# hbaatz/nerf-tex

Hardware: AMD Instinct MI355X
Metric: ray-samples/sec (MLP+composite) at 800x800x64 (higher is better)
Workload: dtype f32; 1 GPU; carpet 800x800x64: 640000 all-hit rays x 64 samples per GPU (BASELINE configs[1]), ParamNerf n_parameters=[1, 6], seeded glorot weights, inputs resident in HBM, fused PE+MLP+composite; rays_per_gpu=640000, hit_rays_total=640000, samples_per_ray=64

## Files before the change

nerf_tex_amd/csrc/ntx_train.hip:

```cpp
#include "nerftex.h"

#include <hip/hip_runtime.h>

#include <algorithm>
#include <cmath>
#include <cstdint>
#include <cstdio>
#include <cstdlib>
#include <cstring>
#include <type_traits>
#include <vector>

#include "ntx_train_device.h"

extern "C" int ntx_set_error(int code, const char *fmt, ...);

#define TRAIN_TRY(expr)                                                                                  \
    do {                                                                                                 \
        hipError_t e_ = (expr);                                                                          \
        if (e_ != hipSuccess) return ntx_set_error(NTX_E_HIP, "%s: %s", #expr, hipGetErrorString(e_)); \
    } while (0)

namespace ntx_train {

constexpr int TM = 128;

struct GemmArgs {
    const float *A; int lda; const float *B; int ldb; float *C; int ldc;
    int M, N, K;
    const float *bias;
    const float *mask; int ldmask;
    int relu, accumulate;
    int k_chunk; long long split_stride;
    float *colsum;
    int aligned;
};

template <int n, bool FAST>
__device__ __forceinline__ void fetch_run(const float *g, bool row_ok, int first, int bound, float *r, bool aligned_ok = false) {
    if (FAST) {
        const f32x4 *v = reinterpret_cast<const f32x4 *>(g);
#pragma unroll
        for (int q = 0; q < n / 4; ++q) { const f32x4 x = v[q]; r[4 * q] = x.x; r[4 * q + 1] = x.y; r[4 * q + 2] = x.z; r[4 * q + 3] = x.w; }
    } else if (row_ok && first + n <= bound && aligned_ok) {
        const f32x4 *v = reinterpret_cast<const f32x4 *>(g);
#pragma unroll
        for (int q = 0; q < n / 4; ++q) { const f32x4 x = v[q]; r[4 * q] = x.x; r[4 * q + 1] = x.y; r[4 * q + 2] = x.z; r[4 * q + 3] = x.w; }
    } else {
#pragma unroll
        for (int q = 0; q < n; ++q) r[q] = (row_ok && first + q < bound) ? g[q] : 0.0f;
    }
}

template <bool A_KCONTIG, int TN_, int TK_>
__device__ __forceinline__ void gemm_body(const GemmArgs &g, int bx, int by, int bz) {
    constexpr int THREADS = TN_ * 2, WCOLS = TN_ / 64, LROWA = TM + 4, LROWB_ = TN_ + 4;
    constexpr int FA = TM * TK_ / THREADS;
    constexpr int FB = TN_ * TK_ / THREADS;
    constexpr int TPR = THREADS / TK_;
    static_assert(FA % 4 == 0 && FB % 4 == 0 && FA * (THREADS / TM) == TK_ && TPR * FB == TN_ && TPR * FA == TM, "panel split");
    __shared__ __attribute__((aligned(16))) float As[2][TK_][LROWA], Bs[2][TK_][LROWB_];
    const int lane = threadIdx.x & 63, wave = threadIdx.x >> 6;
    const int j0 = bx * TN_, i0 = by * TM;
    const int k_begin = bz * g.k_chunk;
    const int k_end = k_begin + g.k_chunk < g.K ? k_begin + g.k_chunk : g.K;
    float *C = g.C + (size_t)bz * (size_t)g.split_stride;
    f32x16 acc[2][2];
#pragma unroll
    for (int a = 0; a < 2; ++a)
#pragma unroll
        for (int b = 0; b < 2; ++b)
#pragma unroll
            for (int r = 0; r < 16; ++r) acc[a][b][r] = 0.0f;
    float ra[2][FA], rb[2][FB], cs[FB];
#pragma unroll
    for (int q = 0; q < FB; ++q) cs[q] = 0.0f;
    const bool want_colsum = !A_KCONTIG && g.colsum != nullptr && by == 0;
    const bool inner = g.aligned && i0 + TM <= g.M && j0 + TN_ <= g.N;
    const int a_row = A_KCONTIG ? (int)(threadIdx.x % TM) : (int)(threadIdx.x / TPR), a_off = A_KCONTIG ? (int)(threadIdx.x / TM) * FA : (int)(threadIdx.x % TPR) * FA;
    const int b_row = (int)(threadIdx.x / TPR), b_off = (int)(threadIdx.x % TPR) * FB;
    auto fetch = [&](int k0, float *fa, float *fb) {
        const bool al = g.aligned != 0;
        if (A_KCONTIG) fetch_run<FA, false>(g.A + (size_t)(i0 + a_row) * g.lda + k0 + a_off, i0 + a_row < g.M, k0 + a_off, k_end, fa, al);
        else fetch_run<FA, false>(g.A + (size_t)(k0 + a_row) * g.lda + i0 + a_off, k0 + a_row < k_end, i0 + a_off, g.M, fa, al);
        fetch_run<FB, false>(g.B + (size_t)(k0 + b_row) * g.ldb + j0 + b_off, k0 + b_row < k_end, j0 + b_off, g.N, fb, al);
    };
    auto stash = [&](int buf, const float *fa, const float *fb) {
        if (want_colsum) {
#pragma unroll
            for (int q = 0; q < FB; ++q) cs[q] += fb[q];
        }
        if (A_KCONTIG) {
#pragma unroll
            for (int q = 0; q < FA; ++q) As[buf][a_off + q][a_row] = fa[q];
        } else {
            f32x4 *d = reinterpret_cast<f32x4 *>(&As[buf][a_row][a_off]);
#pragma unroll
            for (int q = 0; q < FA / 4; ++q) d[q] = f32x4{fa[4 * q], fa[4 * q + 1], fa[4 * q + 2], fa[4 * q + 3]};
        }
        f32x4 *d = reinterpret_cast<f32x4 *>(&Bs[buf][b_row][b_off]);
#pragma unroll
        for (int q = 0; q < FB / 4; ++q) d[q] = f32x4{fb[4 * q], fb[4 * q + 1], fb[4 * q + 2], fb[4 * q + 3]};
    };
    const int n_panels = (k_end - k_begin + TK_ - 1) / TK_;
    const int n_full = inner ? (k_end - k_begin) / TK_ : 0;
    const int wi = (wave / WCOLS) * 64 + 2 * (lane & 31), wj = (wave % WCOLS) * 64 + 2 * (lane & 31), kh = lane >> 5;
    const bool wave_live = j0 + (wave % WCOLS) * 64 < g.N;
    auto compute = [&](int buf) {
        if (!wave_live) return;
        f32x2 av[2], bv[2];
        av[0] = *reinterpret_cast<const f32x2 *>(&As[buf][kh][wi]); bv[0] = *reinterpret_cast<const f32x2 *>(&Bs[buf][kh][wj]);
#pragma unroll
        for (int st = 0; st < TK_ / 2; ++st) {
            const int c = st & 1, n = c ^ 1;
            if (st + 1 < TK_ / 2) {
                const int kk = 2 * (st + 1) + kh;
                av[n] = *reinterpret_cast<const f32x2 *>(&As[buf][kk][wi]); bv[n] = *reinterpret_cast<const f32x2 *>(&Bs[buf][kk][wj]);
            }
            __builtin_amdgcn_sched_barrier(0);
            acc[0][0] = __builtin_amdgcn_mfma_f32_32x32x2f32(av[c].x, bv[c].x, acc[0][0], 0, 0, 0);
            acc[0][1] = __builtin_amdgcn_mfma_f32_32x32x2f32(av[c].x, bv[c].y, acc[0][1], 0, 0, 0);
            acc[1][0] = __builtin_amdgcn_mfma_f32_32x32x2f32(av[c].y, bv[c].x, acc[1][0], 0, 0, 0);
            acc[1][1] = __builtin_amdgcn_mfma_f32_32x32x2f32(av[c].y, bv[c].y, acc[1][1], 0, 0, 0);
            __builtin_amdgcn_sched_barrier(0);
        }
    };
    auto fetch_fast = [&](int k0, float *fa, float *fb) {
        const float *ga = A_KCONTIG ? g.A + (size_t)(i0 + a_row) * g.lda + k0 + a_off : g.A + (size_t)(k0 + a_row) * g.lda + i0 + a_off;
        fetch_run<FA, true>(ga, true, 0, 0, fa);
        fetch_run<FB, true>(g.B + (size_t)(k0 + b_row) * g.ldb + j0 + b_off, true, 0, 0, fb);
    };
    auto pipeline = [&](auto fast_tag, int first, int last) {
        constexpr bool FAST = decltype(fast_tag)::value;
        auto get = [&](int kt, float *fa, float *fb) { if (FAST) fetch_fast(k_begin + kt * TK_, fa, fb); else fetch(k_begin + kt * TK_, fa, fb); };
        if (first >= last) return;
        get(first, ra[0], rb[0]); stash(0, ra[0], rb[0]);
        if (first + 1 < last) get(first + 1, ra[1], rb[1]);
        __syncthreads();
        int kt = first;
        for (; kt + 3 < last; kt += 2) {
            get(kt + 2, ra[0], rb[0]); compute(0); stash(1, ra[1], rb[1]); __syncthreads();
            get(kt + 3, ra[1], rb[1]); compute(1); stash(0, ra[0], rb[0]); __syncthreads();
        }
        for (; kt < last; ++kt) {
            const int buf = (kt - first) & 1;
            if (kt + 2 < last) { if (buf) get(kt + 2, ra[1], rb[1]); else get(kt + 2, ra[0], rb[0]); }
            compute(buf);
            if (kt + 1 < last) { if (buf) stash(0, ra[0], rb[0]); else stash(1, ra[1], rb[1]); }
            __syncthreads();
        }
    };
    pipeline(std::true_type{}, 0, n_full);
    pipeline(std::false_type{}, n_full, n_panels);
    const bool whole = i0 + TM <= g.M && j0 + TN_ <= g.N && (g.ldc % 2 == 0) && (!g.mask || g.ldmask % 2 == 0) && ((uintptr_t)C % 8 == 0) && ((uintptr_t)g.mask % 8 == 0);
    const int j = j0 + (wave % WCOLS) * 64 + 2 * (lane & 31);
    const float bj0 = (g.bias && j < g.N) ? g.bias[j] : 0.0f, bj1 = (g.bias && j + 1 < g.N) ? g.bias[j + 1] : 0.0f;
#pragma unroll
    for (int a = 0; a < 2; ++a)
#pragma unroll
        for (int r = 0; r < 16; ++r) {
            const int i = i0 + (wave / WCOLS) * 64 + 2 * (8 * (r >> 2) + (r & 3) + 4 * kh) + a;
            float v0 = acc[a][0][r], v1 = acc[a][1][r];
            float *c = C + (size_t)i * g.ldc + j;
            if (whole) {
                f32x2 *c2 = reinterpret_cast<f32x2 *>(c);
                if (g.accumulate) { const f32x2 o = *c2; v0 += o.x; v1 += o.y; }
                v0 += bj0; v1 += bj1;
                if (g.relu) { v0 = v0 > 0.0f ? v0 : 0.0f; v1 = v1 > 0.0f ? v1 : 0.0f; }
                if (g.mask) { const f32x2 mk = *reinterpret_cast<const f32x2 *>(g.mask + (size_t)i * g.ldmask + j); if (!(mk.x > 0.0f)) v0 = 0.0f; if (!(mk.y > 0.0f)) v1 = 0.0f; }
                *c2 = f32x2{v0, v1};
            } else if (i < g.M) {
#pragma unroll
                for (int b = 0; b < 2; ++b) {
                    if (j + b >= g.N) continue;
                    float v = b ? v1 : v0;
                    if (g.accumulate) v = v + c[b];
                    v = v + (b ? bj1 : bj0);
                    if (g.relu) v = v > 0.0f ? v : 0.0f;
                    if (g.mask && !(g.mask[(size_t)i * g.ldmask + j + b] > 0.0f)) v = 0.0f;
                    c[b] = v;
                }
            }
        }
    if (want_colsum) {
        float (*red)[LROWB_] = Bs[0];
#pragma unroll
        for (int q = 0; q < FB; ++q) red[b_row][b_off + q] = cs[q];
        __syncthreads();
        if ((int)threadIdx.x < TN_ && j0 + (int)threadIdx.x < g.N) {
            float sum = 0.0f;
            for (int q = 0; q < TK_; ++q) sum += red[q][threadIdx.x];
            g.colsum[(size_t)bz * g.N + j0 + threadIdx.x] = sum;
        }
    }
}


__device__ __forceinline__ void gemm_place(int lin, int nx, int ny, int nz, int &bx, int &by, int &bz) {
    const int tiles = nx * ny;
    if (nz % 8 == 0) {
        const int xcd = lin & 7, slot = lin >> 3, tile = slot % tiles;
        bz = (slot / tiles) * 8 + xcd; bx = tile % nx; by = tile / nx;
    } else { bx = lin % nx; by = (lin / nx) % ny; bz = lin / tiles; }
}
template <bool A_KCONTIG, int TN_, int TK_, int WAVES_PER_EU = 2>
__global__ __launch_bounds__(TN_ * 2) __attribute__((amdgpu_waves_per_eu(WAVES_PER_EU, 8))) void gemm_kernel(GemmArgs g) {
    int bx, by, bz;
    gemm_place(blockIdx.x + gridDim.x * (blockIdx.y + gridDim.y * blockIdx.z), gridDim.x, gridDim.y, gridDim.z, bx, by, bz);
    gemm_body<A_KCONTIG, TN_, TK_>(g, bx, by, bz);
}

constexpr int MAX_REDUCE_BATCH = 32;
struct ReduceJob { const float *partial; int n_split; long long stride, count, pair; float *out; long long first; };
struct ReduceBatch { ReduceJob job[MAX_REDUCE_BATCH]; int n; };
__global__ void reduce_batch_kernel(ReduceBatch b) {
    const long long g = (long long)blockIdx.x * blockDim.x + threadIdx.x;
    int j = 0;
    while (j + 1 < b.n && g >= b.job[j + 1].first) ++j;
    const ReduceJob &r = b.job[j];
    const long long e = g - r.first;
    if (e >= r.count) return;
    float s4[4] = {0.0f, 0.0f, 0.0f, 0.0f};
    auto at = [&](int z) { const float *p = r.partial + (size_t)z * r.stride + e; return r.pair > 0 ? p[0] + p[r.pair] : p[0]; };
    int z = 0;
    for (; z + 4 <= r.n_split; z += 4) {
#pragma unroll
        for (int q = 0; q < 4; ++q) s4[q] += at(z + q);
    }
    for (int q = 0; z < r.n_split; ++z, ++q) s4[q] += at(z);
    r.out[e] = (s4[0] + s4[1]) + (s4[2] + s4[3]);
}

enum { PACK_HIDDEN = 0, PACK_LINEAR = 1, PACK_AUX_ROW = 2, PACK_AUX_RGB = 3, PACK_COPY = 4 };
struct PackSeg {
    const float *src; long long sk, sc;
    int mode;
    int K, ncols, nt;
    float *dst; long long first, count;
};
struct PackArgs { const PackSeg *seg; int n_seg; long long total; };
__global__ void pack_kernel(PackArgs a) {
    const long long e = (long long)blockIdx.x * blockDim.x + threadIdx.x;
    if (e >= a.total) return;
    int lo = 0, hi = a.n_seg - 1;
    while (lo < hi) { const int mid = (lo + hi + 1) >> 1; if (a.seg[mid].first <= e) lo = mid; else hi = mid - 1; }
    const PackSeg &p = a.seg[lo];
    const long long o = e - p.first;
    float v = 0.0f;
    if (p.mode == PACK_COPY) v = p.src[o];
    else if (p.mode == PACK_AUX_ROW) {
        const int h = (int)(o >> 7) & 1, V = (int)(o & 127), k = hidden_row(V, h);
        v = k < p.K ? p.src[k * p.sk] : 0.0f;
    } else if (p.mode == PACK_AUX_RGB) {
        const int c = (int)(o >> 7), h = (int)(o >> 6) & 1, V = (int)(o & 63);
        v = p.src[hidden_row(V, h) * 3 + c];
    } else {
        const int c = (int)(o & 3), lane = (int)((o >> 2) & 63);
        const long long rec = o >> 8;
        const int G = p.nt / 4, g = (int)(rec % G), s = (int)(rec / G);
        const int f = lane & 31, kh = lane >> 5;
        const int k = p.mode == PACK_HIDDEN ? hidden_row(s, kh) : 2 * s + kh, col = 32 * (4 * g + c) + f;
        if (k < p.K && col < p.ncols) v = p.src[k * p.sk + col * p.sc];
    }
    p.dst[o] = v;
}

struct EncodeArgs {
    const float *rays_o, *rays_d, *z, *params, *cone;
    long long rays_per_param_row, M;
    int n_rays, S, n_geo, n_app, pos_freq, dir_freq, param_freq, blur_idx;
    float *posO; int ptiles;
    float *dirO; int dtiles;
    float *dists;
};
__global__ __launch_bounds__(64) void encode_kernel(EncodeArgs a) {
    const int lane = threadIdx.x, n = lane & 31, h = lane >> 5, blk = blockIdx.x, part = blockIdx.y;
    const long long m = (long long)blk * 32 + n;
    const bool valid = m < a.M;
    const int ray = valid ? (int)(m / a.S) : 0, s = valid ? (int)(m - (long long)ray * a.S) : 0;
    const float d[3] = {a.rays_d[3 * ray], a.rays_d[3 * ray + 1], a.rays_d[3 * ray + 2]};
    const float dn = sqrtf((d[0] * d[0] + d[1] * d[1]) + d[2] * d[2]);
    const float zr = a.z[(size_t)ray * a.S + s];
    const bool hit = isfinite(zr);
    const float z = hit ? zr : 0.0f;
    const int P = a.n_geo + a.n_app;
    const float *pr = a.params + (size_t)(ray / a.rays_per_param_row) * (P > 0 ? P : 1);
    auto param = [&](int c) { return c == a.blur_idx ? (hit ? pr[c] * (a.cone[ray] * z) : 0.0f) : pr[c]; };
    float *O = part == 0 ? a.posO : a.dirO;
    const int tiles = part == 0 ? a.ptiles : a.dtiles;
    auto put = [&](int row, float v) {
        if (!valid) v = 0.0f;
        O[(((size_t)blk * tiles + (row >> 5)) * 4 + (n >> 3)) * 256 + ((row & 31) + 32 * ((n >> 2) & 1)) * 4 + (n & 3)] = v;
    };
    auto fourier = [&](int r0, int D, int L, auto x) {
        if (h == 0) for (int c = 0; c < D; ++c) put(r0 + c, x(c));
        for (int f = 0; f < L; ++f)
            for (int c = 0; c < D; ++c) put(r0 + D + 2 * D * f + h * D + c, ntx::sin_q(ldexpf(1.0f, f) * x(c), h));
    };
    if (part == 0) {
        const float o[3] = {a.rays_o[3 * ray], a.rays_o[3 * ray + 1], a.rays_o[3 * ray + 2]};
        fourier(0, 3, a.pos_freq, [&](int c) { return o[c] + d[c] * z; });
        if (a.n_geo > 0) fourier(3 * (1 + 2 * a.pos_freq), a.n_geo, a.param_freq, [&](int c) { return param(c); });
    } else {
        fourier(0, 3, a.dir_freq, [&](int c) { return d[c] / dn; });
        if (a.n_app > 0) fourier(3 * (1 + 2 * a.dir_freq), a.n_app, a.param_freq, [&](int c) { return param(a.n_geo + c); });
        if (valid && h == 0) {
            const float zn = s + 1 < a.S ? a.z[(size_t)ray * a.S + s + 1] : 0.0f;
            const float dist = s + 1 < a.S ? zn - z : (a.S > 1 ? z - a.z[(size_t)ray * a.S + s - 1] : 0.0f);
            a.dists[(size_t)ray * a.S + s] = hit ? dist * dn : 0.0f;
        }
    }
}

__global__ __launch_bounds__(64) void encode_ipe_kernel(EncodeArgs a) {
    const int lane = threadIdx.x, n = lane & 31, h = lane >> 5, blk = blockIdx.x, part = blockIdx.y;
    const long long m = (long long)blk * 32 + n;
    const bool valid = m < a.M;
    const int ray = valid ? (int)(m / a.S) : 0, s = valid ? (int)(m - (long long)ray * a.S) : 0;
    const float d[3] = {a.rays_d[3 * ray], a.rays_d[3 * ray + 1], a.rays_d[3 * ray + 2]};
    const float dn = sqrtf((d[0] * d[0] + d[1] * d[1]) + d[2] * d[2]);
    const float *zr = a.z + (size_t)ray * (a.S + 1) + s;
    const float e0 = zr[0], e1 = zr[1];
    const bool hit = isfinite(e0) && isfinite(e1);
    const int P = a.n_geo + a.n_app;
    const float *pr = a.params + (size_t)(ray / a.rays_per_param_row) * (P + 1);
    auto param = [&](int k) { return pr[k < a.blur_idx ? k : k + 1]; };
    float *O = part == 0 ? a.posO : a.dirO;
    const int tiles = part == 0 ? a.ptiles : a.dtiles;
    auto put = [&](int row, float v) {
        if (!valid) v = 0.0f;
        O[(((size_t)blk * tiles + (row >> 5)) * 4 + (n >> 3)) * 256 + ((row & 31) + 32 * ((n >> 2) & 1)) * 4 + (n & 3)] = v;
    };
    auto fourier = [&](int r0, int D, int L, auto x) {
        if (h == 0) for (int c = 0; c < D; ++c) put(r0 + c, x(c));
        for (int f = 0; f < L; ++f)
            for (int c = 0; c < D; ++c) put(r0 + D + 2 * D * f + h * D + c, ntx::sin_q(ldexpf(1.0f, f) * x(c), h));
    };
    if (part == 0) {
        float mean[3] = {a.rays_o[3 * ray], a.rays_o[3 * ray + 1], a.rays_o[3 * ray + 2]}, cov[3] = {0.0f, 0.0f, 0.0f};
        if (hit) {
            float t_mean, t_var, r_var;
            ntx::cone_moments((e0 + e1) / 2.0f, (e1 - e0) / 2.0f, pr[a.blur_idx] * a.cone[ray], t_mean, t_var, r_var);
            for (int c = 0; c < 3; ++c) mean[c] = mean[c] + d[c] * t_mean;
            ntx::cone_cov(t_var, r_var, d, cov);
        }
        const int L = a.pos_freq;
        for (int f = 0; f < L; ++f)
            for (int c = 0; c < 3; ++c)
                put(h * 3 * L + 3 * f + c, ntx::sin_q(mean[c] * ldexpf(1.0f, f), h) * expf(-0.5f * (cov[c] * ldexpf(1.0f, 2 * f))));
        if (a.n_geo > 0) fourier(6 * L, a.n_geo, a.param_freq, [&](int c) { return param(c); });
    } else {
        fourier(0, 3, a.dir_freq, [&](int c) { return d[c] / dn; });
        if (a.n_app > 0) fourier(3 * (1 + 2 * a.dir_freq), a.n_app, a.param_freq, [&](int c) { return param(a.n_geo + c); });
        if (valid && h == 0) a.dists[(size_t)ray * a.S + s] = hit ? (e1 - e0) * dn : 0.0f;
    }
}

struct DirRowArgs {
    const float *rays_d, *params; long long rays_per_param_row;
    int n_rays, n_geo, n_app, dir_freq, param_freq, Kd, splice;
    const float *w, *bias;
    float *rows;
};
__global__ __launch_bounds__(256) void dirrow_kernel(DirRowArgs a) {
    __shared__ float feat[8 * MAX_PB_GROUPS];
    const int ray = blockIdx.x, f = threadIdx.x;
    const float d[3] = {a.rays_d[3 * ray], a.rays_d[3 * ray + 1], a.rays_d[3 * ray + 2]};
    const float dn = sqrtf((d[0] * d[0] + d[1] * d[1]) + d[2] * d[2]);
    const int P = a.n_geo + a.n_app + (a.splice >= 0 ? 1 : 0);
    const float *pr = a.params + (size_t)(ray / a.rays_per_param_row) * (P > 0 ? P : 1);
    if (f < a.Kd) {
        const int K3 = 3 * (1 + 2 * a.dir_freq);
        const int r = f < K3 ? f : f - K3, D = f < K3 ? 3 : a.n_app;
        auto x = [&](int c) { const int k = a.n_geo + c; return f < K3 ? d[c] / dn : pr[a.splice >= 0 && k >= a.splice ? k + 1 : k]; };
        float v;
        if (r < D) v = x(r);
        else { const int q = r - D, band = q / (2 * D), hc = q - band * 2 * D, hh = hc / D, c = hc - hh * D; v = ntx::sin_q(ldexpf(1.0f, band) * x(c), hh); }
        feat[f] = v;
    }
    __syncthreads();
    float acc = a.bias[f];
    for (int k = 0; k < a.Kd; ++k) acc = fmaf(feat[k], a.w[(size_t)k * 256 + f], acc);
    const int T = f >> 5, g = (f >> 3) & 3, h = (f >> 2) & 1, c = f & 3;
    a.rows[(size_t)ray * 256 + h * 128 + 16 * T + 4 * g + c] = acc;
}

struct CompositeArgs {
    const float *raw_rgb, *sigma, *dists;
    const float *noise;
    int n_rays, S, map_exr, composite_bkgd; float bkgd[3];
    const float *color_true, *alpha_true;
    int kind, loss_fn, alpha_loss_fn, filter_color_loss, use_hard_mask; float gamma;
    float *color, *alpha, *ray_loss;
    float *weights;
    float *dgrad;
    float *dhead;
    long long M;
};
constexpr int MAX_TRAIN_SAMPLES = 1024;
__device__ __forceinline__ float wave_sumf(float v) { for (int o = 32; o > 0; o >>= 1) v += __shfl_xor(v, o); return v; }
__device__ __forceinline__ float rgb_of(float raw, int map_exr) {
    if (map_exr) return raw > 0.0f ? raw + 1.0f : expf(raw);
    return 1.0f / (1.0f + expf(-raw));
}
__device__ __forceinline__ void loss_term(int fn, float t, float p, float inv_n, float &value, float &grad) {
    if (fn == NTX_LOSS_MSE) { const float e = t - p; value = e * e * inv_n; grad = -2.0f * e * inv_n; }
    else {
        const float e = t - p, den = (t + p) + 1e-2f, ae = fabsf(e);
        const float sgn = e > 0.0f ? 1.0f : (e < 0.0f ? -1.0f : 0.0f);
        value = ae / den * inv_n; grad = (-sgn / den - ae / (den * den)) * inv_n;
    }
}
__device__ __forceinline__ size_t dhead_at(long long m, int row) {
    const long long blk = m >> 5; const int p = (int)(m & 31);
    return (size_t)((blk * 4 + (p >> 3)) * 256 + (row + 32 * ((p >> 2) & 1)) * 4 + (p & 3));
}
__global__ __launch_bounds__(256) void composite_loss_kernel(CompositeArgs a) {
    __shared__ float sh_a[4][MAX_TRAIN_SAMPLES], sh_T[4][MAX_TRAIN_SAMPLES];
    const int lane = threadIdx.x & 63, wave = threadIdx.x >> 6;
    if (blockIdx.x == 0) {
        const long long end = (a.M + 31) / 32 * 32;
        for (long long m = a.M + threadIdx.x; m < end; m += 256)
            for (int r = 0; r < 4; ++r) a.dhead[dhead_at(m, r)] = 0.0f;
    }
    const int ray = blockIdx.x * 4 + wave;
    if (ray >= a.n_rays) return;
    const int S = a.S;
    const float *sg = a.sigma + (size_t)ray * S, *ds = a.dists + (size_t)ray * S, *rr = a.raw_rgb + (size_t)ray * S * 3;
    const float *nz = a.noise ? a.noise + (size_t)ray * S : nullptr;
    float *el = sh_a[wave], *T = sh_T[wave];
    for (int s = lane; s < S; s += 64) { const float v = nz ? sg[s] + nz[s] : sg[s]; const float r = v > 0.0f ? v : 0.0f; el[s] = expf(-r * ds[s]); }
    __builtin_amdgcn_wave_barrier();
    float carry = 1.0f;
    for (int s0 = 0; s0 < S; s0 += 64) {
        const int s = s0 + lane;
        float f = s < S ? el[s] + 1e-10f : 1.0f, incl = f;
        for (int o = 1; o < 64; o <<= 1) { const float w = __shfl_up(incl, o); if (lane >= o) incl *= w; }
        float excl = __shfl_up(incl, 1);
        if (lane == 0) excl = 1.0f;
        if (s < S) T[s] = carry * excl;
        carry *= __shfl(incl, 63);
    }
    __builtin_amdgcn_wave_barrier();
    float c0 = 0.0f, c1 = 0.0f, c2 = 0.0f, A = 0.0f;
    for (int s = lane; s < S; s += 64) {
        const float w = (1.0f - el[s]) * T[s];
        c0 += w * rgb_of(rr[3 * s], a.map_exr); c1 += w * rgb_of(rr[3 * s + 1], a.map_exr); c2 += w * rgb_of(rr[3 * s + 2], a.map_exr);
        A += w;
        if (a.weights) a.weights[(size_t)ray * S + s] = w;
    }
    c0 = wave_sumf(c0); c1 = wave_sumf(c1); c2 = wave_sumf(c2); A = wave_sumf(A);
    if (a.composite_bkgd) { c0 += (1.0f - A) * a.bkgd[0]; c1 += (1.0f - A) * a.bkgd[1]; c2 += (1.0f - A) * a.bkgd[2]; }
    const float cp[3] = {c0, c1, c2};
    float dC[3], dA = 0.0f, total = 0.0f;
    {
        const float inv_c = 1.0f / (float)(a.n_rays * 3), inv_a = 1.0f / (float)a.n_rays;
        float mask = 1.0f;
        if (a.kind == NTX_LOSS_ALPHA && a.filter_color_loss) mask = a.use_hard_mask ? (a.alpha_true[ray] > 0.0f ? 1.0f : 0.0f) : a.alpha_true[ray];
        for (int c = 0; c < 3; ++c) {
            float v, gr;
            loss_term(a.loss_fn, a.color_true[3 * ray + c] * mask, cp[c] * mask, inv_c, v, gr);
            total += v; dC[c] = gr * mask;
        }
        if (a.kind == NTX_LOSS_ALPHA) { float v; loss_term(a.alpha_loss_fn, a.alpha_true[ray], A, inv_a, v, dA); total += a.gamma * v; dA *= a.gamma; }
    }
    if (lane == 0) { a.color[3 * ray] = c0; a.color[3 * ray + 1] = c1; a.color[3 * ray + 2] = c2; a.alpha[ray] = A; a.ray_loss[ray] = total; }
    if (a.composite_bkgd) dA -= (dC[0] * a.bkgd[0] + dC[1] * a.bkgd[1]) + dC[2] * a.bkgd[2];
    float Z_carry = 1.0f, V_carry = 0.0f;
    for (int s0 = ((S - 1) / 64) * 64; s0 >= 0; s0 -= 64) {
        const int s = s0 + lane;
        float cs = 0.0f, rgb[3] = {0.0f, 0.0f, 0.0f}, e = 1.0f;
        float F = 1.0f, Bz = 0.0f, Bv = 0.0f;
        if (s < S) {
            e = el[s];
            for (int c = 0; c < 3; ++c) rgb[c] = rgb_of(rr[3 * s + c], a.map_exr);
            cs = (dC[0] * rgb[0] + dC[1] * rgb[1]) + dC[2] * rgb[2];
            F = e + 1e-10f; Bz = -1e-10f; Bv = cs * (1.0f - e);
        }
        for (int o = 1; o < 64; o <<= 1) {
            const float Fo = __shfl_down(F, o), Bzo = __shfl_down(Bz, o), Bvo = __shfl_down(Bv, o);
            if (lane + o < 64) { Bz = fmaf(F, Bzo, Bz); Bv = fmaf(F, Bvo, Bv); F *= Fo; }
        }
        float Fn = __shfl_down(F, 1), Bzn = __shfl_down(Bz, 1), Bvn = __shfl_down(Bv, 1);
        if (lane == 63) { Fn = 1.0f; Bzn = 0.0f; Bvn = 0.0f; }
        const float Z = fmaf(Fn, Z_carry, Bzn), V = fmaf(Fn, V_carry, Bvn);
        if (s < S) {
            const float w = (1.0f - e) * T[s];
            const float d_a = T[s] * fmaf(dA, Z, cs - V);
            const float sig = nz ? sg[s] + nz[s] : sg[s];
            float gr[4];
            for (int c = 0; c < 3; ++c) {
                const float raw = rr[3 * s + c];
                const float drgb = a.map_exr ? (raw > 0.0f ? 1.0f : expf(raw)) : rgb[c] * (1.0f - rgb[c]);
                gr[c] = w * dC[c] * drgb;
            }
            gr[3] = sig > 0.0f ? d_a * ds[s] * e : 0.0f;
            const long long m = (long long)ray * S + s;
            *reinterpret_cast<f32x4 *>(a.dgrad + 4 * m) = f32x4{gr[0], gr[1], gr[2], gr[3]};
            for (int r = 0; r < 4; ++r) a.dhead[dhead_at(m, r)] = gr[r];
        }
        const float F0 = __shfl(F, 0);
        Z_carry = fmaf(F0, Z_carry, __shfl(Bz, 0)); V_carry = fmaf(F0, V_carry, __shfl(Bv, 0));
    }
}
__global__ __launch_bounds__(1024) void loss_sum_kernel(const float *__restrict__ ray_loss, int n_rays, float *__restrict__ loss) {
    __shared__ float red[1024];
    float total = 0.0f;
    for (int r = threadIdx.x; r < n_rays; r += blockDim.x) total += ray_loss[r];
    red[threadIdx.x] = total;
    __syncthreads();
    for (int o = blockDim.x / 2; o > 0; o >>= 1) { if ((int)threadIdx.x < o) red[threadIdx.x] += red[threadIdx.x + o]; __syncthreads(); }
    if (threadIdx.x == 0) *loss = red[0];
}

__global__ void adam_kernel(float *__restrict__ w, const float *__restrict__ g, float *__restrict__ m, float *__restrict__ v, long long n, float lr_t, float b1,
                            float b2, float eps) {
    const long long e = (long long)blockIdx.x * blockDim.x + threadIdx.x;
    if (e >= n) return;
    const float ge = g[e];
    const float me = m[e] + (ge - m[e]) * (1.0f - b1);
    const float ve = v[e] + (ge * ge - v[e]) * (1.0f - b2);
    m[e] = me; v[e] = ve;
    w[e] = w[e] - (me * lr_t) / (sqrtf(ve) + eps);
}

}

struct TLayer { int in, out; size_t w, b; };

struct ntx_trainer {
    int device = 0, cus = 256;
    ntx_model_desc desc{};
    int Kp = 0, Kd = 0, P = 0, ptiles = 0, dtiles = 0, PS = 0, DS = 0;
    bool ipe = false;
    TLayer trunk[8], feature, c1, c2, rgb, alpha;
    size_t n_weights = 0;
    long long cap = 0, cap_blocks = 0, cap_rays = 0;
    float *w = nullptr, *grad = nullptr, *adam_m = nullptr, *adam_v = nullptr;
    float *wfwd = nullptr, *wdx = nullptr, *aux = nullptr; size_t fwd_floats = 0, dx_floats = 0;
    ntx_train::PackSeg *pack_seg = nullptr; int n_pack = 0; long long pack_total = 0;
    float *posO = nullptr, *dirO = nullptr;
    float *act = nullptr; long long act_stride = 0;
    unsigned int *bits = nullptr; long long bits_stride = 0;
    int fwd_variant = 0;
    float *sigma = nullptr, *raw_rgb = nullptr, *z = nullptr, *dists = nullptr, *noise = nullptr;
    float *dirrow = nullptr;
    float *dgrad = nullptr, *dhead = nullptr, *gout = nullptr; long long gout_stride = 0;
    ntx_train::DwJob *jobs = nullptr; int n_jobs = 0; long long total_cost = 0;
    std::vector<ntx_train::DwJob> jobs_host; std::vector<int> reduce_job;
    float *dw_partial = nullptr;
    ntx_train::ReduceBatch reduce{};
    float *color = nullptr, *alpha_out = nullptr, *ray_loss = nullptr, *loss = nullptr;
    float *weights_out = nullptr;
    float *stash = nullptr;
    long long adam_iterations = 0;
};

namespace {

using namespace ntx_train;


void free_all(ntx_trainer *t) {
    if (!t) return;
    (void)hipSetDevice(t->device);
    void *ptrs[] = {t->w, t->grad, t->adam_m, t->adam_v, t->wfwd, t->wdx, t->aux, t->pack_seg, t->posO, t->dirO, t->sigma, t->raw_rgb, t->z, t->dists, t->noise,
                    t->dgrad, t->dhead, t->jobs, t->dw_partial, t->stash, t->dirrow, t->color, t->alpha_out, t->ray_loss, t->loss, t->act, t->bits, t->gout};
    for (void *p : ptrs) if (p) (void)hipFree(p);
    delete t;
}

template <bool AK>
void launch_gemm(hipStream_t st, GemmArgs g) {
    g.k_chunk = g.K;
    g.aligned = (g.lda % 4 == 0) && (g.ldb % 4 == 0) && (((uintptr_t)g.A | (uintptr_t)g.B) % 16 == 0);
    hipLaunchKernelGGL((gemm_kernel<AK, 128, 16>), dim3((g.N + 127) / 128, (g.M + TM - 1) / TM, 1), dim3(256), 0, st, g);
}

}

namespace ntx_train {
template <int K, bool HOIST> void launch_fwd_variant(hipStream_t st, unsigned grid, const FwdArgs &a);
void launch_fwd_chain(int variant, bool hoist, hipStream_t st, unsigned grid, const FwdArgs &a) {
    switch (variant * 2 + (hoist ? 1 : 0)) {
        case 0: launch_fwd_variant<0, false>(st, grid, a); break;
        case 1: launch_fwd_variant<0, true>(st, grid, a); break;
        case 2: launch_fwd_variant<1, false>(st, grid, a); break;
        case 3: launch_fwd_variant<1, true>(st, grid, a); break;
        case 4: launch_fwd_variant<2, false>(st, grid, a); break;
        case 5: launch_fwd_variant<2, true>(st, grid, a); break;
        case 6: launch_fwd_variant<3, false>(st, grid, a); break;
        default: launch_fwd_variant<3, true>(st, grid, a); break;
    }
}
}

extern "C" {

int ntx_sample_depths(const float *t, int64_t n_rays, int n_points, uint32_t flags, uint64_t perturb_seed, const ntx_render_opts *opts, float *z_out,
                      ntx_stream stream);
int ntx_sample_noise(int64_t n_rays, int n_points, uint64_t seed, const ntx_render_opts *opts, float *noise_out, ntx_stream stream);

int ntx_trainer_create(const ntx_model_desc *desc, const float *weights, size_t n_floats, int device, int64_t max_rays, int max_samples_per_ray, ntx_trainer **out) {
    if (!out) return ntx_set_error(NTX_E_INVALID, "out is NULL");
    *out = nullptr;
    if (!desc || !weights) return ntx_set_error(NTX_E_INVALID, "desc / weights is NULL");
    const bool ipe = desc->pos_encoding == NTX_POS_IPE && desc->n_pos == 6;
    if (desc->kind != NTX_MODEL_PARAMNERF || desc->depth != 8 || desc->width != 256 || desc->skip != 4 || desc->color_depth != 1 ||
        !((desc->pos_encoding == NTX_POS_FOURIER && desc->n_pos == 3) || ipe))
        return ntx_set_error(NTX_E_UNSUPPORTED, "training is built for the ParamNerf architecture of the shipped training configs (depth 8, width 256, skips [4], color_depth 1, "
                                                "Fourier features on n_pos 3 or IPE on n_pos 6); others render but do not train");
    if (desc->n_geo < 0 || desc->n_app < 0 || desc->n_geo + desc->n_app > 16) return ntx_set_error(NTX_E_INVALID, "n_parameters out of range");
    if (desc->pos_freq < 0 || desc->dir_freq < 0 || desc->param_freq < 0) return ntx_set_error(NTX_E_INVALID, "negative band count");
    const int Kp = (ipe ? 6 * desc->pos_freq : 3 * (1 + 2 * desc->pos_freq)) + desc->n_geo * (1 + 2 * desc->param_freq), Kd = 3 * (1 + 2 * desc->dir_freq) + desc->n_app * (1 + 2 * desc->param_freq);
    if (Kp > 8 * MAX_PB_GROUPS || Kd > 8 * MAX_PB_GROUPS)
        return ntx_set_error(NTX_E_UNSUPPORTED, "training: pos_map (%d) / dir_map (%d) wider than %d features (the chain holds a block's encoded inputs in registers)", Kp, Kd,
                             8 * MAX_PB_GROUPS);
    if (max_rays < 1 || max_samples_per_ray < 2 || max_samples_per_ray > MAX_TRAIN_SAMPLES || max_rays * (int64_t)max_samples_per_ray > (int64_t)1 << 30)
        return ntx_set_error(NTX_E_INVALID, "max_rays / max_samples_per_ray out of range (samples per ray <= %d)", MAX_TRAIN_SAMPLES);
    int ndev = 0;
    if (hipGetDeviceCount(&ndev) != hipSuccess || ndev <= 0) return ntx_set_error(NTX_E_NODEVICE, "no HIP device visible");
    if (device < 0 || device >= ndev) return ntx_set_error(NTX_E_INVALID, "device %d out of range [0,%d)", device, ndev);
    ntx_trainer *t = new ntx_trainer();
    t->device = device; t->desc = *desc; t->ipe = ipe;
    t->P = desc->n_geo + desc->n_app; t->Kp = Kp; t->Kd = Kd;
    t->ptiles = (Kp + 31) / 32; t->dtiles = (Kd + 31) / 32;
    {
        const int psg = ((Kp + 1) / 2 + 3) / 4, dsg = ((Kd + 1) / 2 + 3) / 4;
        t->fwd_variant = 3;
        for (int v = 2; v >= 0; --v)
            if (FWD_VARIANTS[v][0] >= psg && FWD_VARIANTS[v][1] >= dsg &&
                FWD_VARIANTS[v][0] + FWD_VARIANTS[v][1] <= FWD_VARIANTS[t->fwd_variant][0] + FWD_VARIANTS[t->fwd_variant][1]) t->fwd_variant = v;
        t->PS = 4 * FWD_VARIANTS[t->fwd_variant][0]; t->DS = 4 * FWD_VARIANTS[t->fwd_variant][1];
    }
    size_t p = 0;
    auto take = [&](int in, int o) { TLayer l{in, o, p, p + (size_t)in * o}; p += (size_t)in * o + o; return l; };
    int k = Kp;
    for (int i = 0; i < 8; ++i) { t->trunk[i] = take(k, 256); k = 256 + (i == 4 ? Kp : 0); }
    t->feature = take(256, 256); t->c1 = take(256 + Kd, 256); t->c2 = take(256, 128); t->rgb = take(128, 3); t->alpha = take(256, 1);
    t->n_weights = p;
    if (n_floats != p) { delete t; return ntx_set_error(NTX_E_INVALID, "weights: %zu floats, the model has %zu", n_floats, p); }
    const long long M = (long long)max_rays * max_samples_per_ray, NB = (M + 31) / 32;
    t->cap = M; t->cap_rays = max_rays; t->cap_blocks = NB;
    int rc = hipSetDevice(device) == hipSuccess ? NTX_OK : ntx_set_error(NTX_E_HIP, "hipSetDevice(%d) failed", device);
    if (rc == NTX_OK) { int n = 0; if (hipDeviceGetAttribute(&n, hipDeviceAttributeMultiprocessorCount, device) == hipSuccess && n > 0) t->cus = n; }
    auto alloc = [&](float **d, size_t n, bool zero = false) -> int {
        if (rc != NTX_OK) return rc;
        if (hipMalloc((void **)d, (n ? n : 1) * sizeof(float)) != hipSuccess) return rc = ntx_set_error(NTX_E_HIP, "hipMalloc of %zu floats failed", n);
        if (zero && hipMemset(*d, 0, (n ? n : 1) * sizeof(float)) != hipSuccess) return rc = ntx_set_error(NTX_E_HIP, "hipMemset failed");
        return rc;
    };
    alloc(&t->w, p); alloc(&t->grad, p, true); alloc(&t->adam_m, p, true); alloc(&t->adam_v, p, true);
    alloc(&t->posO, (size_t)NB * t->ptiles * 1024, true); alloc(&t->dirO, (size_t)NB * t->dtiles * 1024, true);
    t->act_stride = t->gout_stride = NB * 8 * 1024; t->bits_stride = NB * 256;
    alloc(&t->act, (size_t)t->act_stride * 11); alloc((float **)&t->bits, (size_t)t->bits_stride * 10); alloc(&t->gout, (size_t)t->gout_stride * 11);
    auto act = [&](int i) { return t->act + (size_t)i * t->act_stride; };
    auto gout = [&](int i) { return t->gout + (size_t)i * t->gout_stride; };
    alloc(&t->sigma, (size_t)M); alloc(&t->raw_rgb, (size_t)M * 3); alloc(&t->z, (size_t)(M + max_rays)); alloc(&t->dists, (size_t)M); alloc(&t->noise, (size_t)M);
    alloc(&t->dirrow, (size_t)max_rays * 256);
    alloc(&t->dgrad, (size_t)NB * 32 * 4); alloc(&t->dhead, (size_t)NB * 1024, true);
    alloc(&t->color, (size_t)max_rays * 3); alloc(&t->alpha_out, (size_t)max_rays); alloc(&t->ray_loss, (size_t)max_rays); alloc(&t->loss, 1);
    if (rc == NTX_OK && hipMemcpy(t->w, weights, p * sizeof(float), hipMemcpyHostToDevice) != hipSuccess) rc = ntx_set_error(NTX_E_HIP, "weight upload failed");
    std::vector<PackSeg> segs;
    long long first = 0;
    auto seg = [&](const float *src, long long sk, long long sc, int mode, int K, int ncols, int nt, size_t *stream_floats, int nsteps) {
        PackSeg s{}; s.src = src; s.sk = sk; s.sc = sc; s.mode = mode; s.K = K; s.ncols = ncols; s.nt = nt;
        const int ring = stream_floats == &t->dx_floats ? DX_RING : RING;
        const long long recs = ((long long)nsteps * (nt / 4) + ring - 1) / ring * ring;
        s.count = recs * 256; s.first = first; s.dst = (float *)(uintptr_t)(*stream_floats * sizeof(float));
        first += s.count; *stream_floats += (size_t)s.count;
        segs.push_back(s);
    };
    const float *W = t->w;
    auto fwd_hidden = [&](const TLayer &l, int row0, int nt) { seg(W + l.w + (size_t)row0 * l.out, l.out, 1, PACK_HIDDEN, 256, l.out, nt, &t->fwd_floats, 128); };
    auto fwd_linear = [&](const TLayer &l, int K, int nsteps) { seg(W + l.w, l.out, 1, PACK_LINEAR, K, l.out, 8, &t->fwd_floats, nsteps); };
    fwd_linear(t->trunk[0], Kp, t->PS);
    for (int i = 1; i < 8; ++i) {
        if (i == 5) { fwd_linear(t->trunk[5], Kp, t->PS); fwd_hidden(t->trunk[5], Kp, 8); }
        else fwd_hidden(t->trunk[i], 0, 8);
    }
    fwd_hidden(t->feature, 0, 8);
    fwd_linear(t->c1, Kd, t->DS); fwd_hidden(t->c1, Kd, 8);
    fwd_hidden(t->c2, 0, 4);
    const size_t n_fwd_segs = segs.size();
    auto dx_hidden = [&](const TLayer &l, int row0, int K, int nsteps) { seg(W + l.w + (size_t)row0 * l.out, 1, l.out, PACK_HIDDEN, K, 256, 8, &t->dx_floats, nsteps); };
    seg(W + t->rgb.w, 1, 3, PACK_LINEAR, 3, 128, 4, &t->dx_floats, 2);
    dx_hidden(t->c2, 0, 128, 64);
    dx_hidden(t->c1, Kd, 256, 128);
    dx_hidden(t->feature, 0, 256, 128);
    seg(W + t->alpha.w, 1, 1, PACK_LINEAR, 1, 256, 8, &t->dx_floats, 1);
    for (int i = 7; i >= 1; --i) dx_hidden(t->trunk[i], i == 5 ? Kp : 0, 256, 128);
    const size_t n_stream_segs = segs.size();
    auto tail = [&](size_t of, size_t *stream_floats) { PackSeg s = segs[of]; s.count = (long long)(stream_floats == &t->dx_floats ? DX_RING : RING) * 256; s.first = first; s.dst = (float *)(uintptr_t)(*stream_floats * sizeof(float));
                                                        first += s.count; *stream_floats += (size_t)s.count; segs.push_back(s); };
    tail(0, &t->fwd_floats); tail(n_fwd_segs, &t->dx_floats);
    auto aux_seg = [&](const float *src, int mode, int K, long long count, size_t at) {
        PackSeg s{}; s.src = src; s.sk = 1; s.mode = mode; s.K = K; s.count = count; s.first = first; s.dst = (float *)(uintptr_t)(at * sizeof(float));
        first += count; segs.push_back(s);
    };
    for (int i = 0; i < 8; ++i) aux_seg(W + t->trunk[i].b, PACK_AUX_ROW, 256, 256, AUX_BIAS + (size_t)i * 256);
    aux_seg(W + t->feature.b, PACK_AUX_ROW, 256, 256, AUX_BIAS + 8 * 256); aux_seg(W + t->c1.b, PACK_AUX_ROW, 256, 256, AUX_BIAS + 9 * 256);
    aux_seg(W + t->c2.b, PACK_AUX_ROW, 128, 256, AUX_BIAS + 10 * 256);
    aux_seg(W + t->alpha.w, PACK_AUX_ROW, 256, 256, AUX_ALPHA_W); aux_seg(W + t->alpha.b, PACK_COPY, 1, 1, AUX_ALPHA_B);
    aux_seg(W + t->rgb.w, PACK_AUX_RGB, 128, 384, AUX_RGB_W); aux_seg(W + t->rgb.b, PACK_COPY, 3, 3, AUX_RGB_B);
    t->pack_total = first; t->n_pack = (int)segs.size();
    alloc(&t->wfwd, t->fwd_floats); alloc(&t->wdx, t->dx_floats); alloc(&t->aux, AUX_FLOATS, true);
    if (rc == NTX_OK) {
        for (size_t i = 0; i < segs.size(); ++i) {
            const bool is_aux = i >= n_stream_segs + 2, is_fwd = i < n_fwd_segs || i == n_stream_segs;
            float *base = is_aux ? t->aux : is_fwd ? t->wfwd : t->wdx;
            segs[i].dst = (float *)((char *)base + (uintptr_t)segs[i].dst);
        }
        if (hipMalloc((void **)&t->pack_seg, segs.size() * sizeof(PackSeg)) != hipSuccess ||
            hipMemcpy(t->pack_seg, segs.data(), segs.size() * sizeof(PackSeg), hipMemcpyHostToDevice) != hipSuccess)
            rc = ntx_set_error(NTX_E_HIP, "segment table upload failed");
    }
    std::vector<DwJob> &jobs = t->jobs_host;
    struct RJ { int job; long long at, count, pair; size_t out; };
    std::vector<RJ> rjobs;
    auto new_job = [&]() { DwJob j{}; for (DwWave &w : j.w) w.shape = -1; jobs.push_back(j); return (int)jobs.size() - 1; };
    auto matrix = [&](int j, int K, int N, size_t g_kernel, long long g_bias, long long *at_bias) {
        const long long at = jobs[j].slot_floats;
        jobs[j].slot_floats += (long long)K * N;
        rjobs.push_back(RJ{j, at, (long long)K * N, 0, g_kernel});
        *at_bias = -1;
        if (g_bias >= 0) { *at_bias = jobs[j].slot_floats; jobs[j].slot_floats += 2 * N; rjobs.push_back(RJ{j, *at_bias, N, N, (size_t)g_bias}); }
        return at;
    };
    auto wave = [&](int j, int w, int shape, const float *A, int rtA, int a0, const float *B, int rtB, int b0, long long at, int K, int N, int c_lo, long long at_bias) {
        DwWave &d = jobs[j].w[w];
        d.A = A; d.rtA = rtA; d.a0 = a0; d.B = B; d.rtB = rtB; d.b0 = b0; d.shape = shape; d.out = at; d.ldc = N; d.row0 = a0 * 32; d.rows_valid = K;
        d.col0 = b0 * 32; d.c_lo = c_lo; d.c_hi = c_lo + N; d.bias_out = a0 == 0 ? at_bias : -1;
        const int cost = shape == 0 ? 256 : shape == 1 ? 198 : 68;
        if (cost > jobs[j].cost) jobs[j].cost = cost;
    };
    auto layer_job = [&](const float *X, const float *dY, size_t g_kernel, size_t g_bias) {
        const int j = new_job(); long long ab; const long long at = matrix(j, 256, 256, g_kernel, (long long)g_bias, &ab);
        for (int w = 0; w < 4; ++w) wave(j, w, 0, X, 8, 4 * (w >> 1), dY, 8, 4 * (w & 1), at, 256, 256, 0, ab);
    };
    {
        const TLayer &r = t->rgb, &al = t->alpha, &c2 = t->c2, &c1 = t->c1, &f = t->feature;
        for (int i = 7; i >= 1; --i) layer_job(act(i - 1), gout(10 - i), t->trunk[i].w + (size_t)(i == 5 ? Kp : 0) * 256, t->trunk[i].b);
        layer_job(act(7), gout(2), f.w, f.b);
        layer_job(act(8), gout(1), c1.w + (size_t)Kd * 256, c1.b);
        {
            const int j = new_job(); long long ab0, ab5;
            const long long at0 = matrix(j, Kp, 256, t->trunk[0].w, (long long)t->trunk[0].b, &ab0), at5 = matrix(j, Kp, 256, t->trunk[5].w, -1, &ab5);
            for (int w = 0; w < 2; ++w) { wave(j, w, 1, t->posO, t->ptiles, 0, gout(10), 8, 4 * w, at0, Kp, 256, 0, ab0); wave(j, 2 + w, 1, t->posO, t->ptiles, 0, gout(5), 8, 4 * w, at5, Kp, 256, 0, ab5); }
        }
        {
            const int j = new_job(); long long abd, ab2;
            const long long atd = matrix(j, Kd, 256, c1.w, -1, &abd), at2 = matrix(j, 256, 128, c2.w, (long long)c2.b, &ab2);
            for (int w = 0; w < 2; ++w) { wave(j, w, 1, t->dirO, t->dtiles, 0, gout(1), 8, 4 * w, atd, Kd, 256, 0, abd); wave(j, 2 + w, 0, act(9), 8, 4 * w, gout(0), 4, 0, at2, 256, 128, 0, ab2); }
        }
        {
            const int j = new_job(); long long abr, aba;
            const long long atr = matrix(j, 128, 3, r.w, (long long)r.b, &abr), ata = matrix(j, 256, 1, al.w, (long long)al.b, &aba);
            wave(j, 0, 2, act(10), 4, 0, t->dhead, 1, 0, atr, 128, 3, 0, abr);
            for (int w = 0; w < 2; ++w) wave(j, 1 + w, 2, act(7), 8, 4 * w, t->dhead, 1, 0, ata, 256, 1, 3, aba);
        }
    }
    t->n_jobs = (int)jobs.size();
    size_t partial_floats = 0;
    for (DwJob &j : jobs) {
        t->total_cost += j.cost;
    }
    for (DwJob &j : jobs) {
        const long long slots = ((long long)j.cost * t->cus + t->total_cost - 1) / t->total_cost + 2;
        j.first_float = (long long)partial_floats; partial_floats += (size_t)(slots * j.slot_floats);
    }
    alloc(&t->dw_partial, partial_floats);
    if (rc == NTX_OK) {
        if (hipMalloc((void **)&t->jobs, jobs.size() * sizeof(DwJob)) != hipSuccess ||
            hipMemcpy(t->jobs, jobs.data(), jobs.size() * sizeof(DwJob), hipMemcpyHostToDevice) != hipSuccess)
            rc = ntx_set_error(NTX_E_HIP, "job table upload failed");
        if ((int)rjobs.size() > MAX_REDUCE_BATCH) rc = ntx_set_error(NTX_E_INVALID, "trainer: too many weight gradients for one launch");
        long long rfirst = 0;
        for (size_t i = 0; i < rjobs.size() && rc == NTX_OK; ++i) {
            ReduceJob &r = t->reduce.job[t->reduce.n++];
            const DwJob &j = jobs[rjobs[i].job];
            r.partial = t->dw_partial + j.first_float + rjobs[i].at; r.n_split = 0; r.stride = j.slot_floats; r.count = rjobs[i].count; r.pair = rjobs[i].pair;
            r.out = t->grad + rjobs[i].out; r.first = rfirst;
            rfirst += (rjobs[i].count + 255) / 256 * 256;
            t->reduce_job.push_back(rjobs[i].job);
        }
    }
    if (rc != NTX_OK) { free_all(t); return rc; }
    *out = t;
    return NTX_OK;
}

int ntx_trainer_destroy(ntx_trainer *t) { free_all(t); return NTX_OK; }

size_t ntx_trainer_weight_count(const ntx_trainer *t) { return t ? t->n_weights : 0; }

static float *trainer_vector(ntx_trainer *t, int what) {
    return what == NTX_TRAINER_WEIGHTS ? t->w : what == NTX_TRAINER_GRADIENTS ? t->grad : what == NTX_TRAINER_ADAM_M ? t->adam_m : what == NTX_TRAINER_ADAM_V ? t->adam_v : nullptr;
}

int ntx_trainer_get(ntx_trainer *t, int what, float *out_host, size_t n_floats) {
    if (!t || !out_host) return ntx_set_error(NTX_E_INVALID, "NULL argument");
    if (n_floats != t->n_weights) return ntx_set_error(NTX_E_INVALID, "%zu floats asked, the model has %zu", n_floats, t->n_weights);
    const float *src = trainer_vector(t, what);
    if (!src) return ntx_set_error(NTX_E_INVALID, "what = %d", what);
    TRAIN_TRY(hipSetDevice(t->device));
    TRAIN_TRY(hipDeviceSynchronize());
    TRAIN_TRY(hipMemcpy(out_host, src, n_floats * sizeof(float), hipMemcpyDeviceToHost));
    return NTX_OK;
}

int ntx_trainer_activation(ntx_trainer *t, int layer, int64_t n_samples_total, float *out_host) {
    if (!t || !out_host) return ntx_set_error(NTX_E_INVALID, "NULL argument");
    if (n_samples_total < 1 || n_samples_total > t->cap) return ntx_set_error(NTX_E_INVALID, "n_samples_total out of range");
    const float *src = nullptr; int tiles = 8;
    auto act = [&](int i) { return t->act + (size_t)i * t->act_stride; };
    auto gout = [&](int i) { return t->gout + (size_t)i * t->gout_stride; };
    if (layer >= 0 && layer < 8) src = act(layer);
    else if (layer == 8) src = act(9);
    else if (layer == 9) { src = act(10); tiles = 4; }
    else if (layer == 10) src = t->sigma;
    else if (layer >= 20 && layer < 28) src = gout(10 - (layer - 20));
    else if (layer == 28) src = gout(1);
    else if (layer == 29) src = gout(2);
    else if (layer == 11) src = t->raw_rgb;
    else if (layer == 30) src = t->dgrad;
    else return ntx_set_error(NTX_E_INVALID, "layer %d (0-7 trunk, 8 / 9 the colour layers, 10 the density, 11 the raw colour; 20-29 the kept gradients, 30 the composite's adjoint)", layer);
    TRAIN_TRY(hipSetDevice(t->device));
    TRAIN_TRY(hipDeviceSynchronize());
    if (layer == 10 || layer == 11 || layer == 30) {
        const size_t width = layer == 10 ? 1 : (layer == 11 ? 3 : 4);
        TRAIN_TRY(hipMemcpy(out_host, src, (size_t)n_samples_total * width * sizeof(float), hipMemcpyDeviceToHost)); return NTX_OK;
    }
    const long long nb = (n_samples_total + 31) / 32;
    std::vector<float> tmp((size_t)nb * tiles * 1024);
    TRAIN_TRY(hipMemcpy(tmp.data(), src, tmp.size() * sizeof(float), hipMemcpyDeviceToHost));
    const int width = tiles * 32;
    for (long long m = 0; m < n_samples_total; ++m) {
        const long long blk = m >> 5; const int p = (int)(m & 31);
        const float *rec = tmp.data() + ((size_t)blk * tiles * 4 + (p >> 3)) * 256 + 32 * ((p >> 2) & 1) * 4 + (p & 3);
        float *o = out_host + (size_t)m * width;
        for (int T = 0; T < tiles; ++T)
            for (int i = 0; i < 32; ++i) o[32 * T + i] = rec[(size_t)T * 1024 + i * 4];
    }
    return NTX_OK;
}

int ntx_trainer_set_weights(ntx_trainer *t, const float *weights_host, size_t n_floats) { return ntx_trainer_set(t, NTX_TRAINER_WEIGHTS, weights_host, n_floats); }

int ntx_trainer_set(ntx_trainer *t, int what, const float *values_host, size_t n_floats) {
    if (!t || !values_host) return ntx_set_error(NTX_E_INVALID, "NULL argument");
    if (n_floats != t->n_weights) return ntx_set_error(NTX_E_INVALID, "%zu floats given, the model has %zu", n_floats, t->n_weights);
    float *dst = trainer_vector(t, what);
    if (!dst) return ntx_set_error(NTX_E_INVALID, "what = %d", what);
    TRAIN_TRY(hipSetDevice(t->device));
    TRAIN_TRY(hipDeviceSynchronize());
    TRAIN_TRY(hipMemcpy(dst, values_host, n_floats * sizeof(float), hipMemcpyHostToDevice));
    return NTX_OK;
}

int ntx_trainer_set_iterations(ntx_trainer *t, int64_t iterations) {
    if (!t || iterations < 0) return ntx_set_error(NTX_E_INVALID, "trainer is NULL or iterations < 0");
    t->adam_iterations = iterations;
    return NTX_OK;
}

int ntx_trainer_composite_weights(ntx_trainer *t, float *weights_dev) {
    if (!t) return ntx_set_error(NTX_E_INVALID, "trainer is NULL");
    if (t->ipe && weights_dev) return ntx_set_error(NTX_E_UNSUPPORTED, "an IPE trainer has no importance pass (MipRenderer: renderer.py:403-404)");
    t->weights_out = weights_dev;
    return NTX_OK;
}

namespace ntx_train {
__global__ void add_kernel(float *__restrict__ dst, const float *__restrict__ src, long long n) {
    const long long e = (long long)blockIdx.x * blockDim.x + threadIdx.x;
    if (e < n) dst[e] += src[e];
}
}

int ntx_trainer_stash_gradients(ntx_trainer *t, int op, ntx_stream stream) {
    if (!t || (op != 0 && op != 1)) return ntx_set_error(NTX_E_INVALID, "trainer is NULL or op is not 0 (keep) / 1 (add back)");
    TRAIN_TRY(hipSetDevice(t->device));
    if (!t->stash) {
        if (op == 1) return ntx_set_error(NTX_E_INVALID, "no gradient was kept");
        TRAIN_TRY(hipMalloc((void **)&t->stash, t->n_weights * sizeof(float)));
    }
    if (op == 0) TRAIN_TRY(hipMemcpyAsync(t->stash, t->grad, t->n_weights * sizeof(float), hipMemcpyDeviceToDevice, (hipStream_t)stream));
    else hipLaunchKernelGGL(ntx_train::add_kernel, dim3((unsigned)((t->n_weights + 255) / 256)), dim3(256), 0, (hipStream_t)stream, t->grad, t->stash, (long long)t->n_weights);
    TRAIN_TRY(hipGetLastError());
    return NTX_OK;
}

int ntx_trainer_device_weights(ntx_trainer *t, const float **weights_dev) {
    if (!t || !weights_dev) return ntx_set_error(NTX_E_INVALID, "NULL argument");
    *weights_dev = t->w;
    return NTX_OK;
}

int ntx_trainer_allreduce_gradients(ntx_trainer *t, ntx_comm *comm, ntx_stream stream) {
    if (!t || !comm) return ntx_set_error(NTX_E_INVALID, "NULL argument");
    return ntx_allreduce_mean_f32(comm, t->grad, t->n_weights, stream);
}

int ntx_train_step_gradients(ntx_trainer *t, const float *rays_o, const float *rays_d, const float *tnear_far, const float *params, int64_t rays_per_param_row,
                             const float *cone_scale, int64_t n_rays, int n_samples, int blur_idx, uint32_t flags, const float *bkgd, uint64_t perturb_seed,
                             const ntx_render_opts *opts, const float *z_vals, const float *color_true, const float *alpha_true, const ntx_loss_desc *loss,
                             float *color_pred, float *alpha_pred, float *loss_out, ntx_stream stream) {
    if (!t) return ntx_set_error(NTX_E_INVALID, "trainer is NULL");
    const int P_in = t->P + (t->ipe ? 1 : 0);
    if (!rays_o || !rays_d || (!tnear_far && !z_vals) || !color_true || !loss || (P_in > 0 && !params)) return ntx_set_error(NTX_E_INVALID, "NULL buffer");
    if (n_rays < 1 || n_rays > t->cap_rays || n_samples < 2 || (long long)n_rays * n_samples > t->cap) return ntx_set_error(NTX_E_INVALID, "n_rays x n_samples beyond what the trainer was created for");
    if (n_samples > MAX_TRAIN_SAMPLES) return ntx_set_error(NTX_E_INVALID, "n_samples > %d", MAX_TRAIN_SAMPLES);
    if (blur_idx >= P_in || (blur_idx >= 0 && !cone_scale) || (t->ipe && blur_idx < 0)) return ntx_set_error(NTX_E_INVALID, "bad blur_idx / cone_scale");
    if (loss->size < sizeof(ntx_loss_desc) || (loss->kind != NTX_LOSS_NERF && loss->kind != NTX_LOSS_ALPHA) || (loss->loss_fn != NTX_LOSS_MSE && loss->loss_fn != NTX_LOSS_SMAPE) ||
        (loss->alpha_loss_fn != NTX_LOSS_MSE && loss->alpha_loss_fn != NTX_LOSS_SMAPE))
        return ntx_set_error(NTX_E_INVALID, "bad ntx_loss_desc");
    if (loss->kind == NTX_LOSS_ALPHA && !alpha_true) return ntx_set_error(NTX_E_INVALID, "AlphaLoss needs alpha_true");
    if (rays_per_param_row < 1) rays_per_param_row = 1;
    TRAIN_TRY(hipSetDevice(t->device));
    hipStream_t st = (hipStream_t)stream;
    const long long M = (long long)n_rays * n_samples;
    const int S = n_samples, n_blocks = (int)((M + 31) / 32);
    {
        PackArgs pa{t->pack_seg, t->n_pack, t->pack_total};
        hipLaunchKernelGGL(pack_kernel, dim3((unsigned)((t->pack_total + 255) / 256)), dim3(256), 0, st, pa);
    }
    const float *z = z_vals;
    if (!z) {
        int rc = ntx_sample_depths(tnear_far, n_rays, t->ipe ? S + 1 : S, flags & NTX_FLAG_PERTURB, perturb_seed, opts, t->z, stream);
        if (rc != NTX_OK) return rc;
        z = t->z;
    }
    const float *noise = nullptr;
    if (flags & NTX_FLAG_RAW_NOISE) {
        int rc = ntx_sample_noise(n_rays, S, perturb_seed, opts, t->noise, stream);
        if (rc != NTX_OK) return rc;
        noise = t->noise;
    }
    {
        EncodeArgs e{}; e.rays_o = rays_o; e.rays_d = rays_d; e.z = z; e.params = params; e.cone = cone_scale; e.rays_per_param_row = rays_per_param_row; e.M = M;
        e.n_rays = (int)n_rays; e.S = S; e.n_geo = t->desc.n_geo; e.n_app = t->desc.n_app; e.pos_freq = t->desc.pos_freq; e.dir_freq = t->desc.dir_freq;
        e.param_freq = t->desc.param_freq; e.blur_idx = blur_idx; e.posO = t->posO; e.ptiles = t->ptiles; e.dirO = t->dirO;
        e.dtiles = t->dtiles; e.dists = t->dists;
        if (t->ipe) hipLaunchKernelGGL(encode_ipe_kernel, dim3((unsigned)n_blocks, 2), dim3(64), 0, st, e);
        else hipLaunchKernelGGL(encode_kernel, dim3((unsigned)n_blocks, 2), dim3(64), 0, st, e);
    }
    const unsigned chain_grid = (unsigned)std::min<long long>(t->cus, (n_blocks + 3) / 4);
    {
        FwdArgs f{}; f.stream = t->wfwd; f.stream_bytes = (uint32_t)(t->fwd_floats * sizeof(float)); f.aux = t->aux; f.M = M;
        f.ptiles = t->ptiles; f.dtiles = t->dtiles; f.pos = t->posO; f.dir = t->dirO;
        f.act = t->act; f.act_stride = t->act_stride; f.bits = t->bits; f.bits_stride = t->bits_stride;
        f.sigma = t->sigma; f.raw_rgb = t->raw_rgb;
        const bool hoist = (t->ipe || blur_idx < 0 || blur_idx < t->desc.n_geo) && S % 32 == 0 && getenv("NERFTEX_TRAIN_NO_DIR_HOIST") == nullptr;
        if (hoist) {
            DirRowArgs dr{}; dr.rays_d = rays_d; dr.params = params; dr.rays_per_param_row = rays_per_param_row; dr.n_rays = (int)n_rays; dr.n_geo = t->desc.n_geo;
            dr.n_app = t->desc.n_app; dr.dir_freq = t->desc.dir_freq; dr.param_freq = t->desc.param_freq; dr.Kd = t->Kd; dr.w = t->w + t->c1.w; dr.bias = t->w + t->c1.b;
            dr.rows = t->dirrow; dr.splice = t->ipe ? blur_idx : -1;
            hipLaunchKernelGGL(dirrow_kernel, dim3((unsigned)n_rays), dim3(256), 0, st, dr);
        }
        f.dirrow = t->dirrow; f.n_rays = (int)n_rays; f.S = S;
        launch_fwd_chain(t->fwd_variant, hoist, st, chain_grid, f);
    }
    {
        CompositeArgs c{};
        c.raw_rgb = t->raw_rgb; c.sigma = t->sigma; c.dists = t->dists; c.noise = noise; c.n_rays = (int)n_rays; c.S = S; c.map_exr = (flags & NTX_FLAG_MAP_EXR) ? 1 : 0;
        c.composite_bkgd = (flags & NTX_FLAG_COMPOSITE_BKGD) ? 1 : 0;
        for (int k = 0; k < 3; ++k) c.bkgd[k] = bkgd ? bkgd[k] : 1.0f;
        c.color_true = color_true; c.alpha_true = alpha_true; c.kind = loss->kind; c.loss_fn = loss->loss_fn; c.alpha_loss_fn = loss->alpha_loss_fn;
        c.filter_color_loss = loss->filter_color_loss; c.use_hard_mask = loss->use_hard_mask; c.gamma = loss->gamma;
        c.weights = t->weights_out;
        c.color = color_pred ? color_pred : t->color; c.alpha = alpha_pred ? alpha_pred : t->alpha_out; c.ray_loss = t->ray_loss; c.dgrad = t->dgrad; c.dhead = t->dhead; c.M = M;
        hipLaunchKernelGGL(composite_loss_kernel, dim3((unsigned)((n_rays + 3) / 4)), dim3(256), 0, st, c);
        hipLaunchKernelGGL(loss_sum_kernel, dim3(1), dim3(1024), 0, st, t->ray_loss, (int)n_rays, loss_out ? loss_out : t->loss);
    }
    {
        DxArgs d{}; d.stream = t->wdx; d.stream_bytes = (uint32_t)(t->dx_floats * sizeof(float)); d.M = M; d.dgrad = t->dgrad;
        d.out = t->gout; d.out_stride = t->gout_stride; d.bits = t->bits; d.bits_stride = t->bits_stride;
        launch_dx_chain(st, chain_grid, d);
    }
    {
        DwArgs d{}; d.jobs = t->jobs; d.n_jobs = t->n_jobs; d.n_blocks = n_blocks; d.total_cost = t->total_cost; d.partial = t->dw_partial;
        const long long G = t->cus, W = t->total_cost * n_blocks;
#ifdef NTX_TRAIN_CLOCKS
        static unsigned long long *clocks = nullptr;
        const size_t nck = (size_t)G * (2 + 3 * t->n_jobs);
        if (getenv("NERFTEX_DW_CLOCKS")) {
            if (!clocks) (void)hipMalloc((void **)&clocks, nck * sizeof(unsigned long long));
            (void)hipMemsetAsync(clocks, 0, nck * sizeof(unsigned long long), st);
            d.clocks = clocks;
        }
#endif
        launch_dw(st, (unsigned)G, d);
#ifdef NTX_TRAIN_CLOCKS
        if (d.clocks) {
            std::vector<unsigned long long> h(nck);
            (void)hipStreamSynchronize(st);
            (void)hipMemcpy(h.data(), clocks, nck * sizeof(unsigned long long), hipMemcpyDeviceToHost);
            unsigned long long t0 = ~0ull;
            for (long long g = 0; g < G; ++g) t0 = std::min(t0, h[g * (2 + 3 * t->n_jobs)]);
            FILE *f = fopen(getenv("NERFTEX_DW_CLOCKS"), "w");
            if (f) {
                for (long long g = 0; g < G; ++g) {
                    const unsigned long long *c = &h[g * (2 + 3 * t->n_jobs)];
                    fprintf(f, "%lld %llu %llu", g, c[0] - t0, c[1] - t0);
                    for (int j = 0; j < t->n_jobs; ++j) if (c[4 + 3 * j]) fprintf(f, "  j%d cost %d blocks %llu %llu-%llu", j, t->jobs_host[j].cost, c[2 + 3 * j], c[3 + 3 * j] - t0, c[4 + 3 * j] - t0);
                    fprintf(f, "\n");
                }
                fclose(f);
            }
        }
#endif
        ReduceBatch rb = t->reduce;
        std::vector<int> slots(t->n_jobs);
        long long start = 0;
        for (int j = 0; j < t->n_jobs; ++j) {
            const long long span = (long long)t->jobs_host[j].cost * n_blocks;
            slots[j] = (int)(dw_last_g(G, W, start, span) - dw_first_g(G, W, start) + 1);
            start += span;
        }
        for (int i = 0; i < rb.n; ++i) rb.job[i].n_split = slots[t->reduce_job[i]];
        const long long total = rb.job[rb.n - 1].first + (rb.job[rb.n - 1].count + 255) / 256 * 256;
        hipLaunchKernelGGL(reduce_batch_kernel, dim3((unsigned)(total / 256)), dim3(256), 0, st, rb);
    }
    TRAIN_TRY(hipGetLastError());
    return NTX_OK;
}

int ntx_trainer_adam_step(ntx_trainer *t, float lrate, float lrate_decay_steps, float lrate_decay_rate, float beta_1, float beta_2, float epsilon, ntx_stream stream) {
    if (!t) return ntx_set_error(NTX_E_INVALID, "trainer is NULL");
    TRAIN_TRY(hipSetDevice(t->device));
    const double step = (double)t->adam_iterations;
    double lr = lrate;
    if (lrate_decay_steps > 0) lr = (double)lrate * std::pow((double)lrate_decay_rate, step / (double)lrate_decay_steps);
    const double tt = step + 1.0;
    const float lr_t = (float)((double)(float)lr * std::sqrt(1.0 - std::pow((double)beta_2, tt)) / (1.0 - std::pow((double)beta_1, tt)));
    hipLaunchKernelGGL(ntx_train::adam_kernel, dim3((unsigned)((t->n_weights + 255) / 256)), dim3(256), 0, (hipStream_t)stream, t->w, t->grad, t->adam_m, t->adam_v,
                       (long long)t->n_weights, lr_t, beta_1, beta_2, epsilon);
    t->adam_iterations += 1;
    TRAIN_TRY(hipGetLastError());
    return NTX_OK;
}

int64_t ntx_trainer_iterations(const ntx_trainer *t) { return t ? t->adam_iterations : -1; }

int ntx_gemm_f32(const float *A, int lda, int a_kcontig, const float *B, int ldb, int b_kcontig, float *C, int ldc, int M, int N, int K, const float *bias, int relu,
                 ntx_stream stream) {
    if (!A || !B || !C || M < 1 || N < 1 || K < 1) return ntx_set_error(NTX_E_INVALID, "bad GEMM arguments");
    ntx_train::GemmArgs g{}; g.A = A; g.lda = lda; g.B = B; g.ldb = ldb; g.C = C; g.ldc = ldc; g.M = M; g.N = N; g.K = K; g.bias = bias; g.relu = relu;
    hipStream_t st = (hipStream_t)stream;
    if (b_kcontig) return ntx_set_error(NTX_E_UNSUPPORTED, "B must be [K][N]");
    if (a_kcontig) launch_gemm<true>(st, g); else launch_gemm<false>(st, g);
    TRAIN_TRY(hipGetLastError());
    return NTX_OK;
}

}
```

nerf_tex_amd/csrc/ntx_train_device.h:

```cpp
#pragma once

#include "ntx_device.h"

namespace ntx_train {

using ntx::f32x16;
using ntx::f32x4;
using ntx::hidden_row;
using ntx::mfma32;
using ntx::RING;
using ntx::static_for;
typedef float f32x2 __attribute__((ext_vector_type(2)));
typedef int i32x4 __attribute__((ext_vector_type(4)));
typedef unsigned int u32x4 __attribute__((ext_vector_type(4)));

#define TRN_DEV __device__ __forceinline__

TRN_DEV __amdgpu_buffer_rsrc_t make_rsrc(const void *base, long long bytes) {
    const long long b = bytes < 0 ? 0 : (bytes > 0x7ffffff0ll ? 0x7ffffff0ll : bytes);
    return __builtin_amdgcn_make_buffer_rsrc(const_cast<void *>(base), 0, (int)b, 0x00020000);
}

TRN_DEV uint32_t o_lane_bytes(int lane) {
    const int n = lane & 31, h = lane >> 5;
    return (uint32_t)((n >> 3) * 1024 + ((n >> 2) & 1) * 512 + h * 64 + (n & 3) * 4);
}
constexpr int STORE_NT = 0;
constexpr uint32_t o_value_bytes(int V) { return (uint32_t)((V >> 4) * 4096 + ((V & 15) >> 2) * 128 + (V & 3) * 16); }

template <int R>
struct WRingT {
    static constexpr int DEPTH = R;
    __amdgpu_buffer_rsrc_t rsrc;
    uint32_t voff;
    f32x4 r[R];
};
typedef WRingT<RING> WRing;
constexpr int DX_RING = 16;
template <class WR>
TRN_DEV f32x4 wr_load(const WR &w, uint32_t byte_off) {
#ifdef NTX_X_WSMALL
    byte_off &= 0xffffu;
#endif
#ifdef NTX_X_NOWLOAD
    if (byte_off >= (uint32_t)WR::DEPTH * 1024u) return w.r[(byte_off >> 10) % WR::DEPTH];
#endif
    return __builtin_bit_cast(f32x4, __builtin_amdgcn_raw_buffer_load_b128(w.rsrc, w.voff, byte_off, 0));
}

template <int NSTEPS, int NMT, bool ZERO, class WR, class Extra>
TRN_DEV void seg_hidden(f32x16 (&acc)[8], WR &ws, uint32_t &sbase, const float (&hin)[128], Extra &&extra) {
    constexpr int RPS = NMT / 4, RING = WR::DEPTH;
    static_assert((NSTEPS * RPS) % RING == 0, "whole ring turns");
    const f32x16 zero = {0.f, 0.f, 0.f, 0.f, 0.f, 0.f, 0.f, 0.f, 0.f, 0.f, 0.f, 0.f, 0.f, 0.f, 0.f, 0.f};
    static_for<NSTEPS>([&](auto S) {
        constexpr int s = S;
        f32x4 w;
        static_for<NMT>([&](auto MT) {
            constexpr int mt = MT;
            if constexpr (mt % 4 == 0) {
                constexpr int rec = s * RPS + mt / 4;
                w = ws.r[rec % RING];
                ws.r[rec % RING] = wr_load(ws, sbase + (uint32_t)(rec + RING) * 1024u);
            }
            if constexpr (ZERO && s == 0) acc[mt] = mfma32(w[mt % 4], hin[s], zero);
            else acc[mt] = mfma32(w[mt % 4], hin[s], acc[mt]);
            extra(S, MT);
            __builtin_amdgcn_sched_barrier(0);
        });
    });
    sbase += (uint32_t)(NSTEPS * RPS) * 1024u;
}

template <int NG, class Fetch>
TRN_DEV void seg_mem(f32x16 (&acc)[8], WRing &ws, uint32_t &sbase, float (&pb)[12], Fetch &&fetch) {
    static_assert(RING == 8, "a group of 4 k-steps of 8 tiles is one ring turn");
    static_for<NG>([&](auto G) {
        constexpr int g = G;
        if constexpr (g + 2 < NG) fetch(std::integral_constant<int, g + 2>{});
        static_for<4>([&](auto K) {
            constexpr int k = K;
            f32x4 w;
            static_for<8>([&](auto MT) {
                constexpr int mt = MT;
                if constexpr (mt % 4 == 0) {
                    constexpr int slot = 2 * k + mt / 4;
                    w = ws.r[slot];
                    ws.r[slot] = wr_load(ws, sbase + (uint32_t)(8 * g + slot + RING) * 1024u);
                }
                acc[mt] = mfma32(w[mt % 4], pb[4 * (g % 3) + k], acc[mt]);
                __builtin_amdgcn_sched_barrier(0);
            });
        });
    });
    sbase += (uint32_t)NG * 8192u;
}

template <int NKS, int NMT, bool ZERO, class WR>
TRN_DEV void seg_few(f32x16 (&acc)[8], WR &ws, uint32_t &sbase, const float (&b)[NKS]) {
    constexpr int RPS = NMT / 4, RING = WR::DEPTH;
    static_assert(NKS * RPS <= RING, "one ring turn");
    const f32x16 zero = {0.f, 0.f, 0.f, 0.f, 0.f, 0.f, 0.f, 0.f, 0.f, 0.f, 0.f, 0.f, 0.f, 0.f, 0.f, 0.f};
    static_for<RING>([&](auto I) {
        constexpr int rec = I;
        const f32x4 w = ws.r[rec];
        ws.r[rec] = wr_load(ws, sbase + (uint32_t)(rec + RING) * 1024u);
        if constexpr (rec < NKS * RPS) {
            constexpr int s = rec / RPS, t0 = 4 * (rec % RPS);
            static_for<4>([&](auto C) {
                constexpr int c = C;
                if constexpr (ZERO && s == 0) acc[t0 + c] = mfma32(w[c], b[s], zero);
                else acc[t0 + c] = mfma32(w[c], b[s], acc[t0 + c]);
                __builtin_amdgcn_sched_barrier(0);
            });
        }
    });
    sbase += (uint32_t)RING * 1024u;
}

template <int V0>
TRN_DEV void convert8_relu_bits(float (&hin)[128], const f32x16 (&prev)[8], uint32_t &w) {
    constexpr int T = V0 >> 4, R = V0 & 15;
    float t0, t1, t2, t3;
    asm("v_accvgpr_read_b32 %0, %13\n\tv_accvgpr_read_b32 %1, %14\n\tv_accvgpr_read_b32 %2, %15\n\tv_accvgpr_read_b32 %3, %16\n\t"
        "v_accvgpr_read_b32 %4, %17\n\tv_accvgpr_read_b32 %5, %18\n\tv_accvgpr_read_b32 %6, %19\n\tv_accvgpr_read_b32 %7, %20\n\t"
        "v_sub_f32 %9, 0, %0\n\tv_sub_f32 %10, 0, %1\n\tv_sub_f32 %11, 0, %2\n\tv_sub_f32 %12, 0, %3\n\t"
        "v_alignbit_b32 %8, %8, %9, 31\n\tv_alignbit_b32 %8, %8, %10, 31\n\tv_alignbit_b32 %8, %8, %11, 31\n\tv_alignbit_b32 %8, %8, %12, 31\n\t"
        "v_sub_f32 %9, 0, %4\n\tv_sub_f32 %10, 0, %5\n\tv_sub_f32 %11, 0, %6\n\tv_sub_f32 %12, 0, %7\n\t"
        "v_alignbit_b32 %8, %8, %9, 31\n\tv_alignbit_b32 %8, %8, %10, 31\n\tv_alignbit_b32 %8, %8, %11, 31\n\tv_alignbit_b32 %8, %8, %12, 31\n\t"
        "v_max_f32 %0, 0, %0\n\tv_max_f32 %1, 0, %1\n\tv_max_f32 %2, 0, %2\n\tv_max_f32 %3, 0, %3\n\t"
        "v_max_f32 %4, 0, %4\n\tv_max_f32 %5, 0, %5\n\tv_max_f32 %6, 0, %6\n\tv_max_f32 %7, 0, %7"
        : "=&v"(hin[V0 + 0]), "=&v"(hin[V0 + 1]), "=&v"(hin[V0 + 2]), "=&v"(hin[V0 + 3]), "=&v"(hin[V0 + 4]), "=&v"(hin[V0 + 5]), "=&v"(hin[V0 + 6]),
          "=&v"(hin[V0 + 7]), "+v"(w), "=&v"(t0), "=&v"(t1), "=&v"(t2), "=&v"(t3)
        : "a"(prev[T][R + 0]), "a"(prev[T][R + 1]), "a"(prev[T][R + 2]), "a"(prev[T][R + 3]), "a"(prev[T][R + 4]), "a"(prev[T][R + 5]), "a"(prev[T][R + 6]),
          "a"(prev[T][R + 7]));
}
constexpr int keep_bit(int V) { return 31 - (V & 31); }

template <int NMT>
TRN_DEV void convert_relu_bits(float (&hin)[128], const f32x16 (&prev)[8], u32x4 &bits) {
    static_for<(NMT + 1) / 2>([&](auto W) {
        constexpr int wd = W;
        uint32_t w = 0;
        static_for<(NMT - 2 * wd >= 2 ? 4 : 2)>([&](auto Q) { convert8_relu_bits<32 * wd + 8 * decltype(Q)::value>(hin, prev, w); });
        bits[wd] = w;
    });
}
template <int NMT>
TRN_DEV void convert_linear(float (&hin)[128], const f32x16 (&prev)[8]) {
    static_for<NMT * 16>([&](auto V) { constexpr int v = V; hin[v] = prev[v >> 4][v & 15]; });
}
template <int NMT>
TRN_DEV void convert_mask(float (&hin)[128], const f32x16 (&prev)[8], const u32x4 &bits) {
    static_for<NMT * 16>([&](auto V) {
        constexpr int v = V;
        const float x = prev[v >> 4][v & 15];
        const int keep = __builtin_amdgcn_sbfe((int)bits[v >> 5], keep_bit(v), 1);
        hin[v] = __builtin_bit_cast(float, __builtin_bit_cast(int, x) & keep);
    });
}

constexpr int AUX_BIAS = 0, AUX_ALPHA_W = 11 * 256, AUX_ALPHA_B = AUX_ALPHA_W + 256, AUX_RGB_W = AUX_ALPHA_B + 4, AUX_RGB_B = AUX_RGB_W + 384,
              AUX_FLOATS = AUX_RGB_B + 4;
template <int MT>
TRN_DEV void bias_tile(f32x16 (&acc)[8], const float *aux, int layer, int h) {
    const f32x4 *b = reinterpret_cast<const f32x4 *>(aux + AUX_BIAS + layer * 256 + h * 128) + MT * 4;
    const f32x4 v0 = b[0], v1 = b[1], v2 = b[2], v3 = b[3];
    acc[MT] = f32x16{v0.x, v0.y, v0.z, v0.w, v1.x, v1.y, v1.z, v1.w, v2.x, v2.y, v2.z, v2.w, v3.x, v3.y, v3.z, v3.w};
}

constexpr int MAX_PB_GROUPS = 12;
struct FwdArgs {
    const float *stream; uint32_t stream_bytes;
    const float *aux;
    long long M;
    int ptiles, dtiles;
    const float *pos, *dir;
    float *act; long long act_stride;
    unsigned int *bits; long long bits_stride;
    float *sigma, *raw_rgb;
    const float *dirrow; int n_rays, S;
};

#ifdef NTX_TRAIN_FWD
template <int PSG, int DSG, bool HOIST>
__global__ __launch_bounds__(256) __attribute__((amdgpu_waves_per_eu(1, 1))) void fwd_chain_kernel(FwdArgs a) {
    __shared__ __attribute__((aligned(16))) float aux_lds[AUX_FLOATS];
    __shared__ __attribute__((aligned(16))) float rows_lds[HOIST ? 4 * 256 : 4];
    ntx::load_aux(aux_lds, a.aux, AUX_FLOATS);
    const int lane = threadIdx.x & 63, n = lane & 31, h = lane >> 5;
    const int wave = __builtin_amdgcn_readfirstlane(blockIdx.x * 4 + (threadIdx.x >> 6)), nwaves = gridDim.x * 4;
    const int n_blocks = (int)((a.M + 31) >> 5);
    if (wave >= n_blocks) return;
    WRing ws;
    ws.rsrc = make_rsrc(a.stream, a.stream_bytes);
    ws.voff = (uint32_t)lane * 16u;
    static_for<RING>([&](auto I) { ws.r[I] = wr_load(ws, (uint32_t)decltype(I)::value * 1024u); });
    const uint32_t lane_o = o_lane_bytes(lane), lane_r = (uint32_t)((n >> 3) * 1024 + ((n >> 2) & 1) * 512 + (n & 3) * 4 + h * 16), lane16 = (uint32_t)lane * 16u;
    float pb[12];
    const __amdgpu_buffer_rsrc_t rs_row = make_rsrc(a.dirrow, HOIST ? (long long)a.n_rays * 1024 : 0);
    __amdgpu_buffer_rsrc_t rs_in = make_rsrc(a.pos + (size_t)wave * a.ptiles * 1024, (long long)a.ptiles * 4096);
    auto fetch = [&](auto G) {
        constexpr int g = G;
        static_for<4>([&](auto K) {
            constexpr int k = K;
            constexpr int s = 4 * g + k;
            pb[4 * (g % 3) + k] = __builtin_bit_cast(float, __builtin_amdgcn_raw_buffer_load_b32(rs_in, lane_r, (uint32_t)((s >> 4) * 4096 + (s & 15) * 32), 0));
        });
    };
    fetch(std::integral_constant<int, 0>{}); fetch(std::integral_constant<int, 1>{});
    for (int blk = wave; blk < n_blocks; blk += nwaves) {
        uint32_t opaque_zero = 0;
        asm volatile("" : "+v"(opaque_zero));
        const float *aux = aux_lds + opaque_zero;
        const float *rows_aux = rows_lds + opaque_zero + (HOIST ? (threadIdx.x >> 6) * 256 : 0) - AUX_BIAS - 9 * 256;
        uint32_t sbase = 0;
        f32x16 acc[8];
        float hin[128];
        const long long m = (long long)blk * 32 + n;
        const bool valid = m < a.M;
        if constexpr (HOIST) {
            const uint32_t ray = __builtin_amdgcn_readfirstlane((int)(((uint32_t)blk * 32u) / (uint32_t)a.S));
            const f32x4 x0 = __builtin_bit_cast(f32x4, __builtin_amdgcn_raw_buffer_load_b128(rs_row, lane16, (ray < (uint32_t)a.n_rays ? ray : (uint32_t)a.n_rays - 1u) * 1024u, 0));
            *reinterpret_cast<f32x4 *>(rows_lds + (threadIdx.x >> 6) * 256 + lane * 4) = x0;
            __builtin_amdgcn_wave_barrier();
        }
        __amdgpu_buffer_rsrc_t rs_out = make_rsrc(a.act, 0);
        auto leaves_to = [&](int idx, int tiles) { rs_out = make_rsrc(a.act + (size_t)idx * a.act_stride + (size_t)blk * tiles * 1024, (long long)tiles * 4096); };
        auto leave = [&](auto V) {
            constexpr int v = V;
#ifndef NTX_X_NOSTORE
            __builtin_amdgcn_raw_buffer_store_b32(__builtin_bit_cast(int, hin[v]), rs_out, lane_o, o_value_bytes(v), STORE_NT);
#endif
        };
        auto bits_leave = [&](int idx, const u32x4 &bw) {
#ifndef NTX_X_NOBITS
            const __amdgpu_buffer_rsrc_t rb = make_rsrc(a.bits + (size_t)idx * a.bits_stride + (size_t)blk * 256, 1024);
            __builtin_amdgcn_raw_buffer_store_b128(__builtin_bit_cast(i32x4, bw), rb, lane16, 0, 0);
#endif
        };
        static_for<8>([&](auto T) { bias_tile<decltype(T)::value>(acc, aux, 0, h); });
        seg_mem<PSG>(acc, ws, sbase, pb, fetch);
        float sig_part = 0.0f;
        auto layer = [&](auto LIc) {
            f32x16 (&cur)[8] = acc; f32x16 (&prev)[8] = acc;
            constexpr int LI = decltype(LIc)::value, in_idx = LI - 1;
            constexpr bool relu_in = in_idx != 8;
            u32x4 bw = {0u, 0u, 0u, 0u};
            if constexpr (HOIST && LI == 9) {
                sbase += (uint32_t)DSG * 8192u;
                static_for<RING>([&](auto I) { ws.r[I] = wr_load(ws, sbase + (uint32_t)decltype(I)::value * 1024u); });
            }
            static_for<4>([&](auto W) {
                constexpr int wd = W;
                if constexpr (relu_in) {
                    uint32_t w = 0;
                    static_for<4>([&](auto Q) { convert8_relu_bits<32 * wd + 8 * decltype(Q)::value>(hin, prev, w); });
                    bw[wd] = w;
                } else static_for<32>([&](auto V) { constexpr int v = 32 * wd + decltype(V)::value; hin[v] = prev[v >> 4][v & 15]; });
                const float *bsrc = (HOIST && LI == 9) ? rows_aux : aux;
                if constexpr (LI < 10 || wd < 2) { bias_tile<2 * wd>(cur, bsrc, LI, h); bias_tile<2 * wd + 1>(cur, bsrc, LI, h); }
            });
            if constexpr (relu_in) bits_leave(in_idx < 8 ? in_idx : 8, bw);
            if constexpr (LI == 8) {
                const f32x4 *wa = reinterpret_cast<const f32x4 *>(aux + AUX_ALPHA_W + h * 128);
                static_for<32>([&](auto I) {
                    constexpr int i = I;
                    const f32x4 w = wa[i];
                    sig_part = __builtin_fmaf(hin[4 * i + 0], w.x, sig_part); sig_part = __builtin_fmaf(hin[4 * i + 1], w.y, sig_part);
                    sig_part = __builtin_fmaf(hin[4 * i + 2], w.z, sig_part); sig_part = __builtin_fmaf(hin[4 * i + 3], w.w, sig_part);
                });
            }
            __builtin_amdgcn_sched_barrier(0);
            leaves_to(in_idx, 8);
            if constexpr (LI == 5) seg_mem<PSG>(cur, ws, sbase, pb, fetch);
            if constexpr (LI == 9 && !HOIST) seg_mem<DSG>(cur, ws, sbase, pb, fetch);
            if constexpr (LI == 4) rs_in = make_rsrc(a.pos + (size_t)blk * a.ptiles * 1024, (long long)a.ptiles * 4096);
            if constexpr (LI == 8 && !HOIST) rs_in = make_rsrc(a.dir + (size_t)blk * a.dtiles * 1024, (long long)a.dtiles * 4096);
            if constexpr (LI == 10) {
                const int nb = blk + nwaves < n_blocks ? blk + nwaves : blk;
                rs_in = make_rsrc(a.pos + (size_t)nb * a.ptiles * 1024, (long long)a.ptiles * 4096);
            }
            auto extra = [&](auto S, auto MT) {
                constexpr int s = decltype(S)::value, mt = decltype(MT)::value;
                if constexpr ((LI == 4 || (LI == 8 && !HOIST) || LI == 10) && mt == 2 && (s == 8 || s == 24)) fetch(std::integral_constant<int, (s == 8 ? 0 : 1)>{});
                if constexpr (mt == 5 || (LI == 10 && mt == 3)) leave(S);
            };
            if constexpr (LI == 10) seg_hidden<128, 4, false>(cur, ws, sbase, hin, extra);
            else seg_hidden<128, 8, false>(cur, ws, sbase, hin, extra);
        };
        static_for<10>([&](auto I) { layer(std::integral_constant<int, decltype(I)::value + 1>{}); });
        {
            u32x4 bw = {0u, 0u, 0u, 0u};
            convert_relu_bits<4>(hin, acc, bw);
            bits_leave(9, bw);
            leaves_to(10, 4);
            static_for<64>([&](auto V) { leave(V); });
            float rgb[3];
            static_for<3>([&](auto C) {
                constexpr int c = C;
                const f32x4 *wc = reinterpret_cast<const f32x4 *>(aux + AUX_RGB_W + (c * 2 + h) * 64);
                float p = 0.0f;
                static_for<16>([&](auto I) {
                    constexpr int i = I;
                    const f32x4 w = wc[i];
                    p = __builtin_fmaf(hin[4 * i + 0], w.x, p); p = __builtin_fmaf(hin[4 * i + 1], w.y, p);
                    p = __builtin_fmaf(hin[4 * i + 2], w.z, p); p = __builtin_fmaf(hin[4 * i + 3], w.w, p);
                });
                rgb[c] = p + __shfl_xor(p, 32, 64) + aux[AUX_RGB_B + c];
            });
            const float sigma = sig_part + __shfl_xor(sig_part, 32, 64) + aux[AUX_ALPHA_B];
            if (valid && h == 0) {
                a.sigma[m] = sigma;
                a.raw_rgb[3 * m + 0] = rgb[0]; a.raw_rgb[3 * m + 1] = rgb[1]; a.raw_rgb[3 * m + 2] = rgb[2];
            }
        }
    }
}

#endif

struct DxArgs {
    const float *stream; uint32_t stream_bytes;
    long long M;
    const float *dgrad;
    float *out; long long out_stride;
    const unsigned int *bits; long long bits_stride;
};

#ifdef NTX_TRAIN_DX
__global__ __launch_bounds__(256) __attribute__((amdgpu_waves_per_eu(1, 1))) void dx_chain_kernel(DxArgs a) {
    const int lane = threadIdx.x & 63, n = lane & 31, h = lane >> 5;
    const int wave = __builtin_amdgcn_readfirstlane(blockIdx.x * 4 + (threadIdx.x >> 6)), nwaves = gridDim.x * 4;
    const int n_blocks = (int)((a.M + 31) >> 5);
    if (wave >= n_blocks) return;
    WRingT<DX_RING> ws;
    ws.rsrc = make_rsrc(a.stream, a.stream_bytes);
    ws.voff = (uint32_t)lane * 16u;
    static_for<DX_RING>([&](auto I) { ws.r[I] = wr_load(ws, (uint32_t)decltype(I)::value * 1024u); });
    const uint32_t lane_o = o_lane_bytes(lane), lane16 = (uint32_t)lane * 16u;
    auto fetch_grad = [&](int blk) {
        const long long m = (long long)blk * 32 + n;
        const f32x4 zero = {0.0f, 0.0f, 0.0f, 0.0f};
        return m < a.M ? *reinterpret_cast<const f32x4 *>(a.dgrad + 4 * m) : zero;
    };
    f32x4 g = fetch_grad(wave);
    for (int blk = wave; blk < n_blocks; blk += nwaves) {
        uint32_t sbase = 0;
        f32x16 acc[8];
        float hin[128];
        __amdgpu_buffer_rsrc_t rs_out = make_rsrc(a.out, 0);
        auto leaves_to = [&](int idx, int tiles) { rs_out = make_rsrc(a.out + (size_t)idx * a.out_stride + (size_t)blk * tiles * 1024, (long long)tiles * 4096); };
        auto leave = [&](auto V) {
            constexpr int v = V;
            __builtin_amdgcn_raw_buffer_store_b32(__builtin_bit_cast(int, hin[v]), rs_out, lane_o, o_value_bytes(v), STORE_NT);
        };
        auto fetch_bits = [&](int idx) {
            const __amdgpu_buffer_rsrc_t rb = make_rsrc(a.bits + (size_t)idx * a.bits_stride + (size_t)blk * 256, 1024);
            return __builtin_bit_cast(u32x4, __builtin_amdgcn_raw_buffer_load_b128(rb, lane16, 0, 0));
        };
        u32x4 bw = fetch_bits(9);
        const float gs = h ? 0.0f : g.w;
        {
            const float b[2] = {h ? g.y : g.x, h ? 0.0f : g.z};
            seg_few<2, 4, true>(acc, ws, sbase, b);
        }
        {
            const int nb = blk + nwaves < n_blocks ? blk + nwaves : blk;
            g = fetch_grad(nb);
        }
        convert_mask<4>(hin, acc, bw);
        bw = fetch_bits(8);
        leaves_to(0, 4);
        seg_hidden<64, 8, true>(acc, ws, sbase, hin, [&](auto S, auto MT) { if constexpr (decltype(MT)::value == 5) leave(S); });
        convert_mask<8>(hin, acc, bw);
        leaves_to(1, 8);
        seg_hidden<128, 8, true>(acc, ws, sbase, hin, [&](auto S, auto MT) { if constexpr (decltype(MT)::value == 5) leave(S); });
        convert_linear<8>(hin, acc);
        static_for<8>([&](auto J) {
            constexpr int j = J;
            bw = fetch_bits(7 - j);
            leaves_to(2 + j, 8);
            seg_hidden<128, 8, true>(acc, ws, sbase, hin, [&](auto S, auto MT) { if constexpr (decltype(MT)::value == 5) leave(S); });
            if constexpr (j == 0) {
                const float b[1] = {gs};
                seg_few<1, 8, false>(acc, ws, sbase, b);
            }
            convert_mask<8>(hin, acc, bw);
        });
        leaves_to(10, 8);
        static_for<128>([&](auto V) { leave(V); });
    }
}

#endif

struct DwWave {
    const float *A; int rtA, a0;
    const float *B; int rtB, b0;
    int shape;
    long long out; int ldc;
    int row0, rows_valid, col0, c_lo, c_hi;
    long long bias_out;
};
struct DwJob { DwWave w[4]; int cost; long long slot_floats, first_float; };
struct DwArgs { const DwJob *jobs; int n_jobs, n_blocks; long long total_cost; float *partial;
                unsigned long long *clocks; };

__host__ __device__ inline long long dw_cut(long long g, long long G, long long W, long long start, long long cost, long long n_blocks) {
    const long long x = g * W / G - start;
    long long b = x <= 0 ? 0 : (x + cost / 2) / cost;
    return b > n_blocks ? n_blocks : b;
}
__host__ __device__ inline long long dw_first_g(long long G, long long W, long long start) { return start * G / W; }
__host__ __device__ inline long long dw_last_g(long long G, long long W, long long start, long long span) { return (start + span - 1) * G / W; }

#ifdef NTX_TRAIN_DW
#ifndef NTX_DW_SYNC
#define NTX_DW_SYNC 16
#endif
constexpr int DW_SYNC = NTX_DW_SYNC;
template <int NA, int NB>
TRN_DEV void dw_piece(const DwWave &tg, float *slot, int blk0, int blk1, int lane) {
    auto uniform_ptr = [](const float *p) {
        const uint32_t lo = (uint32_t)__builtin_amdgcn_readfirstlane((int)(uint32_t)(uintptr_t)p), hi = (uint32_t)__builtin_amdgcn_readfirstlane((int)(uint32_t)((uintptr_t)p >> 32));
        return (const float *)(uintptr_t)(((uint64_t)hi << 32) | (uint64_t)lo);
    };
    const float *A = uniform_ptr(tg.A), *B = uniform_ptr(tg.B);
    const int rtA = __builtin_amdgcn_readfirstlane(tg.rtA), a0 = __builtin_amdgcn_readfirstlane(tg.a0), rtB = __builtin_amdgcn_readfirstlane(tg.rtB), b0 = __builtin_amdgcn_readfirstlane(tg.b0);
    f32x16 acc[NA][NB];
    static_for<NA>([&](auto Ai) { static_for<NB>([&](auto Bi) {
        acc[Ai][Bi] = f32x16{0.f, 0.f, 0.f, 0.f, 0.f, 0.f, 0.f, 0.f, 0.f, 0.f, 0.f, 0.f, 0.f, 0.f, 0.f, 0.f}; }); });
    f32x4 bsum[NB];
    static_for<NB>([&](auto Bi) { bsum[Bi] = f32x4{0.0f, 0.0f, 0.0f, 0.0f}; });
    const bool want_bias = tg.bias_out >= 0;
    const int nblk = blk1 - blk0;
    if (nblk > 0) {
        const __amdgpu_buffer_rsrc_t ra = make_rsrc(A + (size_t)blk0 * rtA * 1024, (long long)nblk * rtA * 4096);
        const __amdgpu_buffer_rsrc_t rb = make_rsrc(B + (size_t)blk0 * rtB * 1024, (long long)nblk * rtB * 4096);
        const uint32_t voff = (uint32_t)lane * 16u;
        const uint32_t stepA = (uint32_t)rtA * 4096u, stepB = (uint32_t)rtB * 4096u, offA = (uint32_t)a0 * 4096u, offB = (uint32_t)b0 * 4096u;
        f32x4 xa[2][NA][2], xb[2][NB][2];
        auto fetch = [&](auto BUF, int i) {
            constexpr int buf = BUF;
#ifdef NTX_X_DWSMALL
            i &= 3;
#endif
#ifdef NTX_X_DWNOLOAD
            if (i > 0) return;
#endif
            const uint32_t oa = (uint32_t)i * stepA + offA + (uint32_t)buf * 2048u, ob = (uint32_t)i * stepB + offB + (uint32_t)buf * 2048u;
            static_for<NA>([&](auto Ai) { static_for<2>([&](auto Q) {
                xa[buf][Ai][Q] = __builtin_bit_cast(f32x4, __builtin_amdgcn_raw_buffer_load_b128(ra, voff, oa + (uint32_t)(decltype(Ai)::value * 4 + decltype(Q)::value) * 1024u, 0)); }); });
            static_for<NB>([&](auto Bi) { static_for<2>([&](auto Q) {
                xb[buf][Bi][Q] = __builtin_bit_cast(f32x4, __builtin_amdgcn_raw_buffer_load_b128(rb, voff, ob + (uint32_t)(decltype(Bi)::value * 4 + decltype(Q)::value) * 1024u, 0)); }); });
        };
        auto compute = [&](auto BUF) {
            constexpr int buf = BUF;
            static_for<2>([&](auto Q) { static_for<4>([&](auto C) {
                constexpr int q = Q, c = C;
                static_for<NA>([&](auto Ai) { static_for<NB>([&](auto Bi) {
                    acc[Ai][Bi] = mfma32(xa[buf][Ai][q][c], xb[buf][Bi][q][c], acc[Ai][Bi]);
                }); });
            }); });
            if (want_bias) static_for<NB>([&](auto Bi) { bsum[Bi] += xb[buf][Bi][0] + xb[buf][Bi][1]; });
        };
        fetch(std::integral_constant<int, 0>{}, 0);
        for (int i = 0; i < nblk; ++i) {
            if ((i & (DW_SYNC - 1)) == 0) __builtin_amdgcn_s_barrier();
            fetch(std::integral_constant<int, 1>{}, i);
            __builtin_amdgcn_sched_barrier(0);
            compute(std::integral_constant<int, 0>{});
            __builtin_amdgcn_sched_barrier(0);
            fetch(std::integral_constant<int, 0>{}, i + 1 < nblk ? i + 1 : i);
            __builtin_amdgcn_sched_barrier(0);
            compute(std::integral_constant<int, 1>{});
            __builtin_amdgcn_sched_barrier(0);
        }
    }
    const int j = lane & 31, hh = lane >> 5;
    const int ldc = __builtin_amdgcn_readfirstlane(tg.ldc), row0 = __builtin_amdgcn_readfirstlane(tg.row0), rows_valid = __builtin_amdgcn_readfirstlane(tg.rows_valid);
    const int col0 = __builtin_amdgcn_readfirstlane(tg.col0), c_lo = __builtin_amdgcn_readfirstlane(tg.c_lo), c_hi = __builtin_amdgcn_readfirstlane(tg.c_hi);
    const long long at_out = (long long)(((uint64_t)(uint32_t)__builtin_amdgcn_readfirstlane((int)(uint32_t)((uint64_t)tg.out >> 32)) << 32) | (uint32_t)__builtin_amdgcn_readfirstlane((int)(uint32_t)(uint64_t)tg.out));
    const __amdgpu_buffer_rsrc_t ro = make_rsrc(slot + at_out, (long long)rows_valid * ldc * 4);
    constexpr uint32_t NOWHERE = 0x7ffffff0u;
    static_for<NB>([&](auto Bi) {
        const int col = col0 + 32 * decltype(Bi)::value + j;
        const bool col_ok = col >= c_lo && col < c_hi;
        const uint32_t coff = (uint32_t)(col - c_lo) * 4u;
        static_for<NA>([&](auto Ai) {
            static_for<16>([&](auto R) {
                constexpr int r = R;
                const int row = row0 + 32 * decltype(Ai)::value + 8 * (r >> 2) + (r & 3) + 4 * hh;
                const uint32_t off = (col_ok && row < rows_valid) ? (uint32_t)(row * ldc) * 4u + coff : NOWHERE;
                __builtin_amdgcn_raw_buffer_store_b32(__builtin_bit_cast(int, (float)acc[Ai][Bi][r]), ro, off, 0, 0);
            });
        });
    });
    if (want_bias) {
        const long long at_bias = (long long)(((uint64_t)(uint32_t)__builtin_amdgcn_readfirstlane((int)(uint32_t)((uint64_t)tg.bias_out >> 32)) << 32) | (uint32_t)__builtin_amdgcn_readfirstlane((int)(uint32_t)(uint64_t)tg.bias_out));
        float *bo = slot + at_bias + (size_t)hh * (c_hi - c_lo);
        static_for<NB>([&](auto Bi) {
            const int col = col0 + 32 * decltype(Bi)::value + j;
            const f32x4 sm = bsum[Bi];
            if (col >= c_lo && col < c_hi) bo[col - c_lo] = (sm.x + sm.y) + (sm.z + sm.w);
        });
    }
}

__global__ __launch_bounds__(256) __attribute__((amdgpu_waves_per_eu(1, 1))) void dw_kernel(DwArgs a) {
    const int lane = threadIdx.x & 63, wave = __builtin_amdgcn_readfirstlane(threadIdx.x >> 6);
    const long long g = blockIdx.x, G = gridDim.x, W = a.total_cost * a.n_blocks;
    long long start = 0;
#ifdef NTX_TRAIN_CLOCKS
    unsigned long long *ck = a.clocks ? a.clocks + (size_t)blockIdx.x * (2 + 3 * a.n_jobs) : nullptr;
    if (ck && threadIdx.x == 0) ck[0] = wall_clock64();
#endif
    for (int jn = 0; jn < a.n_jobs; ++jn) {
        const DwJob &job = a.jobs[jn];
        const long long cost = job.cost, span = cost * a.n_blocks;
        const long long g0 = dw_first_g(G, W, start), g1 = dw_last_g(G, W, start, span);
        if (__builtin_amdgcn_readfirstlane((int)(g >= g0 && g <= g1))) {
            const int blk0 = __builtin_amdgcn_readfirstlane((int)dw_cut(g, G, W, start, cost, a.n_blocks)), blk1 = __builtin_amdgcn_readfirstlane((int)dw_cut(g + 1, G, W, start, cost, a.n_blocks));
            const DwWave &wv = job.w[wave];
            const int shape = __builtin_amdgcn_readfirstlane(wv.shape);
            const int my_slot = __builtin_amdgcn_readfirstlane((int)(g - g0));
            float *slot = a.partial + job.first_float + (long long)my_slot * job.slot_floats;
#ifdef NTX_TRAIN_CLOCKS
            const unsigned long long c0 = wall_clock64();
#endif
            if (shape == 0) dw_piece<4, 4>(wv, slot, blk0, blk1, lane);
            else if (shape == 1) dw_piece<3, 4>(wv, slot, blk0, blk1, lane);
            else if (shape == 2) dw_piece<4, 1>(wv, slot, blk0, blk1, lane);
            else for (int i = 0; i < blk1 - blk0; i += DW_SYNC) __builtin_amdgcn_s_barrier();
#ifdef NTX_TRAIN_CLOCKS
            __syncthreads();
            if (ck && threadIdx.x == 0) { ck[2 + 3 * jn] = (unsigned long long)(blk1 - blk0); ck[3 + 3 * jn] = c0; ck[4 + 3 * jn] = wall_clock64(); }
#endif
        }
        start += span;
    }
#ifdef NTX_TRAIN_CLOCKS
    if (ck && threadIdx.x == 0) ck[1] = wall_clock64();
#endif
}
#endif

constexpr int FWD_VARIANTS[4][2] = {{9, 11}, {9, 8}, {11, 8}, {MAX_PB_GROUPS, MAX_PB_GROUPS}};
void launch_fwd_chain(int variant, bool hoist, hipStream_t st, unsigned grid, const FwdArgs &a);
void launch_dx_chain(hipStream_t st, unsigned grid, const DxArgs &a);
void launch_dw(hipStream_t st, unsigned grid, const DwArgs &a);

}
```

Baseline: 112.7 million ray-samples/s.

## Fold linear feature layer into colour layer weights to drop one GEMM

The feature layer has no activation before the colour layer, so the two are merged: a small matmul kernel computes W_fold = W_feature·W_c1h and a folded bias each step. The forward and dx chains then run one fewer 256x256 layer, which also frees one activation and one gradient buffer. Weight gradients for the original feature and c1 layers are recovered afterwards with extra small matmuls, and the debug readback for layer 29 is rebuilt on the host. The change also adds an empty asm clobber of a255 in the chain kernels to reserve the accumulator register file. The cost is a few extra tiny kernel launches per step and the rounding differences that come from reassociating the product.

```diff
diff --git a/nerf_tex_amd/csrc/ntx_train.hip b/nerf_tex_amd/csrc/ntx_train.hip
--- a/nerf_tex_amd/csrc/ntx_train.hip
+++ b/nerf_tex_amd/csrc/ntx_train.hip
@@ -265,6 +265,34 @@
     p.dst[o] = v;
 }
 
+constexpr int MAX_FOLD_JOBS = 3;
+struct FoldJob { const float *A; int sai, sak; const float *B; int sbk, sbj; const float *C0, *u, *v; float *C; int M; };
+struct FoldBatch { FoldJob job[MAX_FOLD_JOBS]; };
+__global__ __launch_bounds__(256) void fold_mm_kernel(FoldBatch b) {
+    __shared__ float As[16][17], Bs[16][17];
+    const FoldJob &g = b.job[blockIdx.y];
+    const int i0 = (int)(blockIdx.x >> 4) * 16, j0 = (int)(blockIdx.x & 15) * 16;
+    if (i0 >= g.M) return;
+    const int ty = threadIdx.x >> 4, tx = threadIdx.x & 15;
+    const int ai = g.sak == 1 ? ty : tx, ak = g.sak == 1 ? tx : ty, bk = g.sbj == 1 ? ty : tx, bj = g.sbj == 1 ? tx : ty;
+    const bool a_ok = i0 + ai < g.M;
+    const float *pa = g.A + (long long)(i0 + ai) * g.sai + (long long)ak * g.sak, *pb = g.B + (long long)bk * g.sbk + (long long)(j0 + bj) * g.sbj;
+    float acc = 0.0f;
+    for (int k0 = 0; k0 < 256; k0 += 16) {
+        As[ai][ak] = a_ok ? pa[(long long)k0 * g.sak] : 0.0f;
+        Bs[bk][bj] = pb[(long long)k0 * g.sbk];
+        __syncthreads();
+#pragma unroll
+        for (int k = 0; k < 16; ++k) acc = fmaf(As[ty][k], Bs[k][tx], acc);
+        __syncthreads();
+    }
+    const int i = i0 + ty, j = j0 + tx;
+    if (i >= g.M) return;
+    if (g.C0) acc += g.C0[j];
+    if (g.u) acc = fmaf(g.u[i], g.v[j], acc);
+    g.C[(long long)i * 256 + j] = acc;
+}
+
 struct EncodeArgs {
     const float *rays_o, *rays_d, *z, *params, *cone;
     long long rays_per_param_row, M;
@@ -538,6 +566,7 @@
     long long cap = 0, cap_blocks = 0, cap_rays = 0;
     float *w = nullptr, *grad = nullptr, *adam_m = nullptr, *adam_v = nullptr;
     float *wfwd = nullptr, *wdx = nullptr, *aux = nullptr; size_t fwd_floats = 0, dx_floats = 0;
+    float *wfold = nullptr, *bfold = nullptr, *dwfold = nullptr;
     ntx_train::PackSeg *pack_seg = nullptr; int n_pack = 0; long long pack_total = 0;
     float *posO = nullptr, *dirO = nullptr;
     float *act = nullptr; long long act_stride = 0;
@@ -564,7 +593,7 @@
 void free_all(ntx_trainer *t) {
     if (!t) return;
     (void)hipSetDevice(t->device);
-    void *ptrs[] = {t->w, t->grad, t->adam_m, t->adam_v, t->wfwd, t->wdx, t->aux, t->pack_seg, t->posO, t->dirO, t->sigma, t->raw_rgb, t->z, t->dists, t->noise,
+    void *ptrs[] = {t->w, t->grad, t->adam_m, t->adam_v, t->wfwd, t->wdx, t->aux, t->wfold, t->bfold, t->dwfold, t->pack_seg, t->posO, t->dirO, t->sigma, t->raw_rgb, t->z, t->dists, t->noise,
                     t->dgrad, t->dhead, t->jobs, t->dw_partial, t->stash, t->dirrow, t->color, t->alpha_out, t->ray_loss, t->loss, t->act, t->bits, t->gout};
     for (void *p : ptrs) if (p) (void)hipFree(p);
     delete t;
@@ -651,9 +680,10 @@
         return rc;
     };
     alloc(&t->w, p); alloc(&t->grad, p, true); alloc(&t->adam_m, p, true); alloc(&t->adam_v, p, true);
+    alloc(&t->wfold, 256 * 256, true); alloc(&t->bfold, 256, true); alloc(&t->dwfold, 256 * 256, true);
     alloc(&t->posO, (size_t)NB * t->ptiles * 1024, true); alloc(&t->dirO, (size_t)NB * t->dtiles * 1024, true);
     t->act_stride = t->gout_stride = NB * 8 * 1024; t->bits_stride = NB * 256;
-    alloc(&t->act, (size_t)t->act_stride * 11); alloc((float **)&t->bits, (size_t)t->bits_stride * 10); alloc(&t->gout, (size_t)t->gout_stride * 11);
+    alloc(&t->act, (size_t)t->act_stride * 10); alloc((float **)&t->bits, (size_t)t->bits_stride * 10); alloc(&t->gout, (size_t)t->gout_stride * 10);
     auto act = [&](int i) { return t->act + (size_t)i * t->act_stride; };
     auto gout = [&](int i) { return t->gout + (size_t)i * t->gout_stride; };
     alloc(&t->sigma, (size_t)M); alloc(&t->raw_rgb, (size_t)M * 3); alloc(&t->z, (size_t)(M + max_rays)); alloc(&t->dists, (size_t)M); alloc(&t->noise, (size_t)M);
@@ -679,15 +709,14 @@
         if (i == 5) { fwd_linear(t->trunk[5], Kp, t->PS); fwd_hidden(t->trunk[5], Kp, 8); }
         else fwd_hidden(t->trunk[i], 0, 8);
     }
-    fwd_hidden(t->feature, 0, 8);
-    fwd_linear(t->c1, Kd, t->DS); fwd_hidden(t->c1, Kd, 8);
+    fwd_linear(t->c1, Kd, t->DS);
+    seg(t->wfold, 256, 1, PACK_HIDDEN, 256, 256, 8, &t->fwd_floats, 128);
     fwd_hidden(t->c2, 0, 4);
     const size_t n_fwd_segs = segs.size();
     auto dx_hidden = [&](const TLayer &l, int row0, int K, int nsteps) { seg(W + l.w + (size_t)row0 * l.out, 1, l.out, PACK_HIDDEN, K, 256, 8, &t->dx_floats, nsteps); };
     seg(W + t->rgb.w, 1, 3, PACK_LINEAR, 3, 128, 4, &t->dx_floats, 2);
     dx_hidden(t->c2, 0, 128, 64);
-    dx_hidden(t->c1, Kd, 256, 128);
-    dx_hidden(t->feature, 0, 256, 128);
+    seg(t->wfold, 1, 256, PACK_HIDDEN, 256, 256, 8, &t->dx_floats, 128);
     seg(W + t->alpha.w, 1, 1, PACK_LINEAR, 1, 256, 8, &t->dx_floats, 1);
     for (int i = 7; i >= 1; --i) dx_hidden(t->trunk[i], i == 5 ? Kp : 0, 256, 128);
     const size_t n_stream_segs = segs.size();
@@ -699,7 +728,7 @@
         first += count; segs.push_back(s);
     };
     for (int i = 0; i < 8; ++i) aux_seg(W + t->trunk[i].b, PACK_AUX_ROW, 256, 256, AUX_BIAS + (size_t)i * 256);
-    aux_seg(W + t->feature.b, PACK_AUX_ROW, 256, 256, AUX_BIAS + 8 * 256); aux_seg(W + t->c1.b, PACK_AUX_ROW, 256, 256, AUX_BIAS + 9 * 256);
+    aux_seg(t->bfold, PACK_AUX_ROW, 256, 256, AUX_BIAS + 9 * 256);
     aux_seg(W + t->c2.b, PACK_AUX_ROW, 128, 256, AUX_BIAS + 10 * 256);
     aux_seg(W + t->alpha.w, PACK_AUX_ROW, 256, 256, AUX_ALPHA_W); aux_seg(W + t->alpha.b, PACK_COPY, 1, 1, AUX_ALPHA_B);
     aux_seg(W + t->rgb.w, PACK_AUX_RGB, 128, 384, AUX_RGB_W); aux_seg(W + t->rgb.b, PACK_COPY, 3, 3, AUX_RGB_B);
@@ -716,15 +745,15 @@
             rc = ntx_set_error(NTX_E_HIP, "segment table upload failed");
     }
     std::vector<DwJob> &jobs = t->jobs_host;
-    struct RJ { int job; long long at, count, pair; size_t out; };
+    struct RJ { int job; long long at, count, pair; size_t out; float *scratch; };
     std::vector<RJ> rjobs;
     auto new_job = [&]() { DwJob j{}; for (DwWave &w : j.w) w.shape = -1; jobs.push_back(j); return (int)jobs.size() - 1; };
-    auto matrix = [&](int j, int K, int N, size_t g_kernel, long long g_bias, long long *at_bias) {
+    auto matrix = [&](int j, int K, int N, size_t g_kernel, long long g_bias, long long *at_bias, float *scratch = nullptr) {
         const long long at = jobs[j].slot_floats;
         jobs[j].slot_floats += (long long)K * N;
-        rjobs.push_back(RJ{j, at, (long long)K * N, 0, g_kernel});
+        rjobs.push_back(RJ{j, at, (long long)K * N, 0, g_kernel, scratch});
         *at_bias = -1;
-        if (g_bias >= 0) { *at_bias = jobs[j].slot_floats; jobs[j].slot_floats += 2 * N; rjobs.push_back(RJ{j, *at_bias, N, N, (size_t)g_bias}); }
+        if (g_bias >= 0) { *at_bias = jobs[j].slot_floats; jobs[j].slot_floats += 2 * N; rjobs.push_back(RJ{j, *at_bias, N, N, (size_t)g_bias, nullptr}); }
         return at;
     };
     auto wave = [&](int j, int w, int shape, const float *A, int rtA, int a0, const float *B, int rtB, int b0, long long at, int K, int N, int c_lo, long long at_bias) {
@@ -734,29 +763,28 @@
         const int cost = shape == 0 ? 256 : shape == 1 ? 198 : 68;
         if (cost > jobs[j].cost) jobs[j].cost = cost;
     };
-    auto layer_job = [&](const float *X, const float *dY, size_t g_kernel, size_t g_bias) {
-        const int j = new_job(); long long ab; const long long at = matrix(j, 256, 256, g_kernel, (long long)g_bias, &ab);
+    auto layer_job = [&](const float *X, const float *dY, size_t g_kernel, size_t g_bias, float *scratch = nullptr) {
+        const int j = new_job(); long long ab; const long long at = matrix(j, 256, 256, g_kernel, (long long)g_bias, &ab, scratch);
         for (int w = 0; w < 4; ++w) wave(j, w, 0, X, 8, 4 * (w >> 1), dY, 8, 4 * (w & 1), at, 256, 256, 0, ab);
     };
     {
-        const TLayer &r = t->rgb, &al = t->alpha, &c2 = t->c2, &c1 = t->c1, &f = t->feature;
-        for (int i = 7; i >= 1; --i) layer_job(act(i - 1), gout(10 - i), t->trunk[i].w + (size_t)(i == 5 ? Kp : 0) * 256, t->trunk[i].b);
-        layer_job(act(7), gout(2), f.w, f.b);
-        layer_job(act(8), gout(1), c1.w + (size_t)Kd * 256, c1.b);
+        const TLayer &r = t->rgb, &al = t->alpha, &c2 = t->c2, &c1 = t->c1;
+        for (int i = 7; i >= 1; --i) layer_job(act(i - 1), gout(9 - i), t->trunk[i].w + (size_t)(i == 5 ? Kp : 0) * 256, t->trunk[i].b);
+        layer_job(act(7), gout(1), 0, c1.b, t->dwfold);
         {
             const int j = new_job(); long long ab0, ab5;
             const long long at0 = matrix(j, Kp, 256, t->trunk[0].w, (long long)t->trunk[0].b, &ab0), at5 = matrix(j, Kp, 256, t->trunk[5].w, -1, &ab5);
-            for (int w = 0; w < 2; ++w) { wave(j, w, 1, t->posO, t->ptiles, 0, gout(10), 8, 4 * w, at0, Kp, 256, 0, ab0); wave(j, 2 + w, 1, t->posO, t->ptiles, 0, gout(5), 8, 4 * w, at5, Kp, 256, 0, ab5); }
+            for (int w = 0; w < 2; ++w) { wave(j, w, 1, t->posO, t->ptiles, 0, gout(9), 8, 4 * w, at0, Kp, 256, 0, ab0); wave(j, 2 + w, 1, t->posO, t->ptiles, 0, gout(4), 8, 4 * w, at5, Kp, 256, 0, ab5); }
         }
         {
             const int j = new_job(); long long abd, ab2;
             const long long atd = matrix(j, Kd, 256, c1.w, -1, &abd), at2 = matrix(j, 256, 128, c2.w, (long long)c2.b, &ab2);
-            for (int w = 0; w < 2; ++w) { wave(j, w, 1, t->dirO, t->dtiles, 0, gout(1), 8, 4 * w, atd, Kd, 256, 0, abd); wave(j, 2 + w, 0, act(9), 8, 4 * w, gout(0), 4, 0, at2, 256, 128, 0, ab2); }
+            for (int w = 0; w < 2; ++w) { wave(j, w, 1, t->dirO, t->dtiles, 0, gout(1), 8, 4 * w, atd, Kd, 256, 0, abd); wave(j, 2 + w, 0, act(8), 8, 4 * w, gout(0), 4, 0, at2, 256, 128, 0, ab2); }
         }
         {
             const int j = new_job(); long long abr, aba;
             const long long atr = matrix(j, 128, 3, r.w, (long long)r.b, &abr), ata = matrix(j, 256, 1, al.w, (long long)al.b, &aba);
-            wave(j, 0, 2, act(10), 4, 0, t->dhead, 1, 0, atr, 128, 3, 0, abr);
+            wave(j, 0, 2, act(9), 4, 0, t->dhead, 1, 0, atr, 128, 3, 0, abr);
             for (int w = 0; w < 2; ++w) wave(j, 1 + w, 2, act(7), 8, 4 * w, t->dhead, 1, 0, ata, 256, 1, 3, aba);
         }
     }
@@ -780,7 +808,7 @@
             ReduceJob &r = t->reduce.job[t->reduce.n++];
             const DwJob &j = jobs[rjobs[i].job];
             r.partial = t->dw_partial + j.first_float + rjobs[i].at; r.n_split = 0; r.stride = j.slot_floats; r.count = rjobs[i].count; r.pair = rjobs[i].pair;
-            r.out = t->grad + rjobs[i].out; r.first = rfirst;
+            r.out = rjobs[i].scratch ? rjobs[i].scratch : t->grad + rjobs[i].out; r.first = rfirst;
             rfirst += (rjobs[i].count + 255) / 256 * 256;
             t->reduce_job.push_back(rjobs[i].job);
         }
@@ -816,12 +844,11 @@
     auto act = [&](int i) { return t->act + (size_t)i * t->act_stride; };
     auto gout = [&](int i) { return t->gout + (size_t)i * t->gout_stride; };
     if (layer >= 0 && layer < 8) src = act(layer);
-    else if (layer == 8) src = act(9);
-    else if (layer == 9) { src = act(10); tiles = 4; }
+    else if (layer == 8) src = act(8);
+    else if (layer == 9) { src = act(9); tiles = 4; }
     else if (layer == 10) src = t->sigma;
-    else if (layer >= 20 && layer < 28) src = gout(10 - (layer - 20));
-    else if (layer == 28) src = gout(1);
-    else if (layer == 29) src = gout(2);
+    else if (layer >= 20 && layer < 28) src = gout(9 - (layer - 20));
+    else if (layer == 28 || layer == 29) src = gout(1);
     else if (layer == 11) src = t->raw_rgb;
     else if (layer == 30) src = t->dgrad;
     else return ntx_set_error(NTX_E_INVALID, "layer %d (0-7 trunk, 8 / 9 the colour layers, 10 the density, 11 the raw colour; 20-29 the kept gradients, 30 the composite's adjoint)", layer);
@@ -841,6 +868,22 @@
         float *o = out_host + (size_t)m * width;
         for (int T = 0; T < tiles; ++T)
             for (int i = 0; i < 32; ++i) o[32 * T + i] = rec[(size_t)T * 1024 + i * 4];
+    }
+    if (layer == 29) {
+        std::vector<float> wh((size_t)256 * 256);
+        TRAIN_TRY(hipMemcpy(wh.data(), t->w + t->c1.w + (size_t)t->Kd * 256, wh.size() * sizeof(float), hipMemcpyDeviceToHost));
+        for (long long m = 0; m < n_samples_total; ++m) {
+            float *o = out_host + (size_t)m * 256;
+            int nz[256], n_nz = 0; double gv[256]; float df[256];
+            for (int j = 0; j < 256; ++j) if (o[j] != 0.0f) { nz[n_nz] = j; gv[n_nz++] = o[j]; }
+            for (int k = 0; k < 256; ++k) {
+                const float *row = wh.data() + (size_t)k * 256;
+                double sum = 0.0;
+                for (int q = 0; q < n_nz; ++q) sum += gv[q] * (double)row[nz[q]];
+                df[k] = (float)sum;
+            }
+            memcpy(o, df, sizeof(df));
+        }
     }
     return NTX_OK;
 }
@@ -921,7 +964,12 @@
     hipStream_t st = (hipStream_t)stream;
     const long long M = (long long)n_rays * n_samples;
     const int S = n_samples, n_blocks = (int)((M + 31) / 32);
+    const float *Wf = t->w + t->feature.w, *bf = t->w + t->feature.b, *Wh = t->w + t->c1.w + (size_t)t->Kd * 256;
     {
+        FoldBatch fb{};
+        fb.job[0] = FoldJob{Wf, 256, 1, Wh, 256, 1, nullptr, nullptr, nullptr, t->wfold, 256};
+        fb.job[1] = FoldJob{bf, 0, 1, Wh, 256, 1, t->w + t->c1.b, nullptr, nullptr, t->bfold, 1};
+        hipLaunchKernelGGL(fold_mm_kernel, dim3(256, 2), dim3(256), 0, st, fb);
         PackArgs pa{t->pack_seg, t->n_pack, t->pack_total};
         hipLaunchKernelGGL(pack_kernel, dim3((unsigned)((t->pack_total + 255) / 256)), dim3(256), 0, st, pa);
     }
@@ -954,7 +1002,7 @@
         const bool hoist = (t->ipe || blur_idx < 0 || blur_idx < t->desc.n_geo) && S % 32 == 0 && getenv("NERFTEX_TRAIN_NO_DIR_HOIST") == nullptr;
         if (hoist) {
             DirRowArgs dr{}; dr.rays_d = rays_d; dr.params = params; dr.rays_per_param_row = rays_per_param_row; dr.n_rays = (int)n_rays; dr.n_geo = t->desc.n_geo;
-            dr.n_app = t->desc.n_app; dr.dir_freq = t->desc.dir_freq; dr.param_freq = t->desc.param_freq; dr.Kd = t->Kd; dr.w = t->w + t->c1.w; dr.bias = t->w + t->c1.b;
+            dr.n_app = t->desc.n_app; dr.dir_freq = t->desc.dir_freq; dr.param_freq = t->desc.param_freq; dr.Kd = t->Kd; dr.w = t->w + t->c1.w; dr.bias = t->bfold;
             dr.rows = t->dirrow; dr.splice = t->ipe ? blur_idx : -1;
             hipLaunchKernelGGL(dirrow_kernel, dim3((unsigned)n_rays), dim3(256), 0, st, dr);
         }
@@ -1021,6 +1069,12 @@
         for (int i = 0; i < rb.n; ++i) rb.job[i].n_split = slots[t->reduce_job[i]];
         const long long total = rb.job[rb.n - 1].first + (rb.job[rb.n - 1].count + 255) / 256 * 256;
         hipLaunchKernelGGL(reduce_batch_kernel, dim3((unsigned)(total / 256)), dim3(256), 0, st, rb);
+        float *dbp = t->grad + t->c1.b;
+        FoldBatch fb{};
+        fb.job[0] = FoldJob{t->dwfold, 256, 1, Wh, 1, 256, nullptr, nullptr, nullptr, t->grad + t->feature.w, 256};
+        fb.job[1] = FoldJob{dbp, 0, 1, Wh, 1, 256, nullptr, nullptr, nullptr, t->grad + t->feature.b, 1};
+        fb.job[2] = FoldJob{Wf, 1, 256, t->dwfold, 256, 1, nullptr, bf, dbp, t->grad + t->c1.w + (size_t)t->Kd * 256, 256};
+        hipLaunchKernelGGL(fold_mm_kernel, dim3(256, 3), dim3(256), 0, st, fb);
     }
     TRAIN_TRY(hipGetLastError());
     return NTX_OK;
diff --git a/nerf_tex_amd/csrc/ntx_train_device.h b/nerf_tex_amd/csrc/ntx_train_device.h
--- a/nerf_tex_amd/csrc/ntx_train_device.h
+++ b/nerf_tex_amd/csrc/ntx_train_device.h
@@ -15,6 +15,8 @@
 typedef unsigned int u32x4 __attribute__((ext_vector_type(4)));
 
 #define TRN_DEV __device__ __forceinline__
+
+TRN_DEV void claim_accumulator_file() { asm volatile("" ::: "a255"); }
 
 TRN_DEV __amdgpu_buffer_rsrc_t make_rsrc(const void *base, long long bytes) {
     const long long b = bytes < 0 ? 0 : (bytes > 0x7ffffff0ll ? 0x7ffffff0ll : bytes);
@@ -147,10 +149,6 @@
     });
 }
 template <int NMT>
-TRN_DEV void convert_linear(float (&hin)[128], const f32x16 (&prev)[8]) {
-    static_for<NMT * 16>([&](auto V) { constexpr int v = V; hin[v] = prev[v >> 4][v & 15]; });
-}
-template <int NMT>
 TRN_DEV void convert_mask(float (&hin)[128], const f32x16 (&prev)[8], const u32x4 &bits) {
     static_for<NMT * 16>([&](auto V) {
         constexpr int v = V;
@@ -163,8 +161,8 @@
 constexpr int AUX_BIAS = 0, AUX_ALPHA_W = 11 * 256, AUX_ALPHA_B = AUX_ALPHA_W + 256, AUX_RGB_W = AUX_ALPHA_B + 4, AUX_RGB_B = AUX_RGB_W + 384,
               AUX_FLOATS = AUX_RGB_B + 4;
 template <int MT>
-TRN_DEV void bias_tile(f32x16 (&acc)[8], const float *aux, int layer, int h) {
-    const f32x4 *b = reinterpret_cast<const f32x4 *>(aux + AUX_BIAS + layer * 256 + h * 128) + MT * 4;
+TRN_DEV void bias_tile(f32x16 (&acc)[8], const float *row, int h) {
+    const f32x4 *b = reinterpret_cast<const f32x4 *>(row + h * 128) + MT * 4;
     const f32x4 v0 = b[0], v1 = b[1], v2 = b[2], v3 = b[3];
     acc[MT] = f32x16{v0.x, v0.y, v0.z, v0.w, v1.x, v1.y, v1.z, v1.w, v2.x, v2.y, v2.z, v2.w, v3.x, v3.y, v3.z, v3.w};
 }
@@ -187,6 +185,7 @@
 __global__ __launch_bounds__(256) __attribute__((amdgpu_waves_per_eu(1, 1))) void fwd_chain_kernel(FwdArgs a) {
     __shared__ __attribute__((aligned(16))) float aux_lds[AUX_FLOATS];
     __shared__ __attribute__((aligned(16))) float rows_lds[HOIST ? 4 * 256 : 4];
+    claim_accumulator_file();
     ntx::load_aux(aux_lds, a.aux, AUX_FLOATS);
     const int lane = threadIdx.x & 63, n = lane & 31, h = lane >> 5;
     const int wave = __builtin_amdgcn_readfirstlane(blockIdx.x * 4 + (threadIdx.x >> 6)), nwaves = gridDim.x * 4;
@@ -213,7 +212,7 @@
         uint32_t opaque_zero = 0;
         asm volatile("" : "+v"(opaque_zero));
         const float *aux = aux_lds + opaque_zero;
-        const float *rows_aux = rows_lds + opaque_zero + (HOIST ? (threadIdx.x >> 6) * 256 : 0) - AUX_BIAS - 9 * 256;
+        const float *ray_row = rows_lds + opaque_zero + (HOIST ? (threadIdx.x >> 6) * 256 : 0);
         uint32_t sbase = 0;
         f32x16 acc[8];
         float hin[128];
@@ -239,13 +238,12 @@
             __builtin_amdgcn_raw_buffer_store_b128(__builtin_bit_cast(i32x4, bw), rb, lane16, 0, 0);
 #endif
         };
-        static_for<8>([&](auto T) { bias_tile<decltype(T)::value>(acc, aux, 0, h); });
+        static_for<8>([&](auto T) { bias_tile<decltype(T)::value>(acc, aux + AUX_BIAS, h); });
         seg_mem<PSG>(acc, ws, sbase, pb, fetch);
         float sig_part = 0.0f;
         auto layer = [&](auto LIc) {
             f32x16 (&cur)[8] = acc; f32x16 (&prev)[8] = acc;
-            constexpr int LI = decltype(LIc)::value, in_idx = LI - 1;
-            constexpr bool relu_in = in_idx != 8;
+            constexpr int LI = decltype(LIc)::value, in_idx = LI < 9 ? LI - 1 : LI - 2;
             u32x4 bw = {0u, 0u, 0u, 0u};
             if constexpr (HOIST && LI == 9) {
                 sbase += (uint32_t)DSG * 8192u;
@@ -253,16 +251,14 @@
             }
             static_for<4>([&](auto W) {
                 constexpr int wd = W;
-                if constexpr (relu_in) {
-                    uint32_t w = 0;
-                    static_for<4>([&](auto Q) { convert8_relu_bits<32 * wd + 8 * decltype(Q)::value>(hin, prev, w); });
-                    bw[wd] = w;
-                } else static_for<32>([&](auto V) { constexpr int v = 32 * wd + decltype(V)::value; hin[v] = prev[v >> 4][v & 15]; });
-                const float *bsrc = (HOIST && LI == 9) ? rows_aux : aux;
-                if constexpr (LI < 10 || wd < 2) { bias_tile<2 * wd>(cur, bsrc, LI, h); bias_tile<2 * wd + 1>(cur, bsrc, LI, h); }
+                uint32_t w = 0;
+                static_for<4>([&](auto Q) { convert8_relu_bits<32 * wd + 8 * decltype(Q)::value>(hin, prev, w); });
+                bw[wd] = w;
+                const float *bsrc = (HOIST && LI == 9) ? ray_row : aux + AUX_BIAS + LI * 256;
+                if constexpr (LI < 10 || wd < 2) { bias_tile<2 * wd>(cur, bsrc, h); bias_tile<2 * wd + 1>(cur, bsrc, h); }
             });
-            if constexpr (relu_in) bits_leave(in_idx < 8 ? in_idx : 8, bw);
-            if constexpr (LI == 8) {
+            bits_leave(in_idx, bw);
+            if constexpr (LI == 9) {
                 const f32x4 *wa = reinterpret_cast<const f32x4 *>(aux + AUX_ALPHA_W + h * 128);
                 static_for<32>([&](auto I) {
                     constexpr int i = I;
@@ -276,25 +272,25 @@
             if constexpr (LI == 5) seg_mem<PSG>(cur, ws, sbase, pb, fetch);
             if constexpr (LI == 9 && !HOIST) seg_mem<DSG>(cur, ws, sbase, pb, fetch);
             if constexpr (LI == 4) rs_in = make_rsrc(a.pos + (size_t)blk * a.ptiles * 1024, (long long)a.ptiles * 4096);
-            if constexpr (LI == 8 && !HOIST) rs_in = make_rsrc(a.dir + (size_t)blk * a.dtiles * 1024, (long long)a.dtiles * 4096);
+            if constexpr (LI == 7 && !HOIST) rs_in = make_rsrc(a.dir + (size_t)blk * a.dtiles * 1024, (long long)a.dtiles * 4096);
             if constexpr (LI == 10) {
                 const int nb = blk + nwaves < n_blocks ? blk + nwaves : blk;
                 rs_in = make_rsrc(a.pos + (size_t)nb * a.ptiles * 1024, (long long)a.ptiles * 4096);
             }
             auto extra = [&](auto S, auto MT) {
                 constexpr int s = decltype(S)::value, mt = decltype(MT)::value;
-                if constexpr ((LI == 4 || (LI == 8 && !HOIST) || LI == 10) && mt == 2 && (s == 8 || s == 24)) fetch(std::integral_constant<int, (s == 8 ? 0 : 1)>{});
+                if constexpr ((LI == 4 || (LI == 7 && !HOIST) || LI == 10) && mt == 2 && (s == 8 || s == 24)) fetch(std::integral_constant<int, (s == 8 ? 0 : 1)>{});
                 if constexpr (mt == 5 || (LI == 10 && mt == 3)) leave(S);
             };
             if constexpr (LI == 10) seg_hidden<128, 4, false>(cur, ws, sbase, hin, extra);
             else seg_hidden<128, 8, false>(cur, ws, sbase, hin, extra);
         };
-        static_for<10>([&](auto I) { layer(std::integral_constant<int, decltype(I)::value + 1>{}); });
+        static_for<9>([&](auto I) { constexpr int i = I; layer(std::integral_constant<int, (i < 7 ? i + 1 : i + 2)>{}); });
         {
             u32x4 bw = {0u, 0u, 0u, 0u};
             convert_relu_bits<4>(hin, acc, bw);
             bits_leave(9, bw);
-            leaves_to(10, 4);
+            leaves_to(9, 4);
             static_for<64>([&](auto V) { leave(V); });
             float rgb[3];
             static_for<3>([&](auto C) {
@@ -330,6 +326,7 @@
 
 #ifdef NTX_TRAIN_DX
 __global__ __launch_bounds__(256) __attribute__((amdgpu_waves_per_eu(1, 1))) void dx_chain_kernel(DxArgs a) {
+    claim_accumulator_file();
     const int lane = threadIdx.x & 63, n = lane & 31, h = lane >> 5;
     const int wave = __builtin_amdgcn_readfirstlane(blockIdx.x * 4 + (threadIdx.x >> 6)), nwaves = gridDim.x * 4;
     const int n_blocks = (int)((a.M + 31) >> 5);
@@ -374,13 +371,10 @@
         leaves_to(0, 4);
         seg_hidden<64, 8, true>(acc, ws, sbase, hin, [&](auto S, auto MT) { if constexpr (decltype(MT)::value == 5) leave(S); });
         convert_mask<8>(hin, acc, bw);
-        leaves_to(1, 8);
-        seg_hidden<128, 8, true>(acc, ws, sbase, hin, [&](auto S, auto MT) { if constexpr (decltype(MT)::value == 5) leave(S); });
-        convert_linear<8>(hin, acc);
         static_for<8>([&](auto J) {
             constexpr int j = J;
             bw = fetch_bits(7 - j);
-            leaves_to(2 + j, 8);
+            leaves_to(1 + j, 8);
             seg_hidden<128, 8, true>(acc, ws, sbase, hin, [&](auto S, auto MT) { if constexpr (decltype(MT)::value == 5) leave(S); });
             if constexpr (j == 0) {
                 const float b[1] = {gs};
@@ -388,7 +382,7 @@
             }
             convert_mask<8>(hin, acc, bw);
         });
-        leaves_to(10, 8);
+        leaves_to(9, 8);
         static_for<128>([&](auto V) { leave(V); });
     }
 }
```

Result: no change. 112.5 million ray-samples/s (-0.2%).
